# ylsung/vl-merging

Hardware: AMD Instinct MI355X
Metric: VL samples/sec (fwd+bwd) base_vl 384^2 at 1/2/4/8 GPUs; merge GB/s vs HBM peak (higher is better)
Workload: dtype bf16

## Files before the change

### include/vlm_hip.h

```cpp
#ifndef VLM_HIP_H
#define VLM_HIP_H
#include <stddef.h>
#include <stdint.h>

#ifdef __cplusplus
extern "C" {
#endif

#define VLM_OK 0
#define VLM_ERR_ARG (-1)
#define VLM_ERR_LAUNCH (-2)
#define VLM_ERR_WORKSPACE (-3)
#define VLM_ERR_UNSUPPORTED (-4)

#define VLM_ABI_VERSION 11
int vlm_abi_version(void);
int vlm_device_cus(void);
int vlm_set_cu_budget(int cus);
int vlm_debug_occupy(int workgroups, int threads, int lds_bytes, int microseconds, void* stream);

#define VLM_MERGE_LERP 0
#define VLM_MERGE_TASKVEC 1
#define VLM_MERGE_MEAN 2
#define VLM_MERGE_MAX_SRC 4
// ... 197 lines not shown
  uint64_t chunks_off;
  uint64_t first_off;
  uint64_t records_off;
  uint64_t results_off;
} vlm_stock_header_t;
#define VLM_STOCK_SUMS (VLM_MERGE_MAX_SRC + VLM_PAIRSTATS_PAIRS)

typedef struct {
  double sq[VLM_MERGE_MAX_SRC];
  double dot[6];
  double cos_pair[6];
  double cos;
  double t;
  float scale;
  uint32_t reserved;
} vlm_stock_result_t;

size_t vlm_stock_plan_bytes(int n_jobs, uint64_t total_elems);
int vlm_stock_plan_upload(const vlm_stock_job_t* jobs_host, int n_jobs, void* workspace, size_t workspace_bytes, void* stream);
int vlm_stock_run(void* workspace, void* stream);

typedef struct {
  void* dst;
  const void* base;
  const void* src[VLM_MERGE_MAX_SRC];
  uint64_t k;
  uint64_t n_elem;
  int32_t n_src;
  float lam;
} vlm_sce_job_t;

typedef struct {
  uint64_t n_jobs, n_units, n_chunks;
  uint64_t jobs_off;
  uint64_t chunks_off;
  uint64_t unit0_off;
  uint64_t units_off;
  uint64_t state_off;
  uint64_t counters_off;
  uint64_t hist_off;
  uint64_t first_off;
  uint64_t records_off;
} vlm_sce_header_t;
typedef struct {
  uint32_t key;
  uint32_t reserved;
  uint64_t rank;
  double sq[VLM_MERGE_MAX_SRC];
  double tot;
  float w[VLM_MERGE_MAX_SRC];
} vlm_sce_result_t;
#define VLM_SCE_COUNTERS 3

size_t vlm_sce_plan_bytes(int n_jobs, uint64_t total_elems);
int vlm_sce_plan_upload(const vlm_sce_job_t* jobs_host, int n_jobs, void* workspace, size_t workspace_bytes, void* stream);
int vlm_sce_run(void* workspace, void* stream);

#define VLM_ACT_NONE 0
#define VLM_ACT_GELU 1
#define VLM_ACT_GELU_BWD 2
#define VLM_ACT_GELU_DERIV 3
#define VLM_ACT_MUL_AUX 4

typedef struct {
  const float* bias;
  const float* col_scale;
  const float* row_scale;
  const float* residual;
  int64_t ld_res;
  void* aux;
  int64_t ld_aux;
  int32_t act;
  float alpha;
  int32_t accumulate;
  int32_t reserved;
  float* col_sum;
  float* col_sum_ws;
  float* splitk_ws;
  uint64_t splitk_ws_bytes;
} vlm_epilogue_t;

int vlm_gemm_bf16(int ta, int tb, int M, int N, int K, const void* A, int lda, const void* B, int ldb, void* C,
                  int ldc, int c_is_f32, const vlm_epilogue_t* epi, void* stream);
#define VLM_GEMM_MAX_GROUPS 4
typedef struct {
  int32_t row0, rows;
  const void* B;
  int32_t ldb;
  int32_t reserved;
  const float* bias;
  float* col_sum;
  float* col_sum_ws;
} vlm_gemm_group_t;
int vlm_gemm_bf16_grouped(int n_groups, const vlm_gemm_group_t* groups, int N, int K, const void* A, int lda, void* C,
                          int ldc, int c_is_f32, const vlm_epilogue_t* epi, void* stream);
typedef struct {
  int32_t row0, rows;
  float* C;
  int32_t accumulate;
  int32_t reserved;
} vlm_wgrad_group_t;
int vlm_gemm_wgrad_grouped(int n_groups, const vlm_wgrad_group_t* groups, int M, int N, const void* A, int lda,
                           const void* B, int ldb, int ldc, float* splitk_ws, uint64_t splitk_ws_bytes, void* stream);
typedef struct {
  const void* dy;
  int32_t ld_dy, M;
  const void* x;
  int32_t ld_x, N;
  float* dW;
  int32_t ldc, accumulate;
} vlm_wgrad_problem_t;
int vlm_gemm_wgrad_batch(int n, const vlm_wgrad_problem_t* problems, int T, float* splitk_ws, uint64_t splitk_ws_bytes,
                         void* stream);
int vlm_gemm_set_big_tile_mode(int mode);

int vlm_layernorm_fwd(const float* x, int ldx, int M, int D, const float* gamma, const float* beta, float eps,
                      void* y, int ldy, int y_is_f32, float* stats, void* stream);
#define VLM_ROW_WS_BYTES(D) ((size_t)1536 * 2 * (size_t)(D) * sizeof(float))
int vlm_layernorm_bwd(const void* dy, int lddy, int dy_is_f32, const float* x, int ldx, const float* stats,
                      const float* gamma, int M, int D, const float* dres, int lddres, float* dx, int lddx,
                      float* dgamma, float* dbeta, float* workspace, size_t workspace_bytes, int* deferred_blocks,
                      void* stream);
typedef struct {
  const void* y;
  int32_t ldy;
  const float* gamma;
  const float* row_scale;
  void* dy;
  int32_t lddy;
  float* dgamma;
  float* dbias;
  float* workspace;
  size_t workspace_bytes;
} vlm_layerscale_t;
int vlm_layernorm_bwd_scale(const void* dy, int lddy, int dy_is_f32, const float* x, int ldx, const float* stats,
                            const float* gamma, int M, int D, const float* dres, int lddres, float* dx, int lddx,
                            float* dgamma, float* dbeta, float* workspace, size_t workspace_bytes,
                            const vlm_layerscale_t* scale, int* deferred_blocks, void* stream);
#define VLM_MAX_FOLD_JOBS 16
typedef struct {
  const float* partials;
  int32_t nblocks;
  int32_t D;
  float* out0;
  float* out1;
} vlm_fold_job_t;
int vlm_colreduce_batch(const vlm_fold_job_t* jobs_host, int n_jobs, void* stream);
int vlm_layerscale_bwd(const float* dx, int lddx, const void* y_bf16, int ldy, const float* gamma,
                       const float* row_scale, int M, int D, void* dy_bf16, int lddy, float* dgamma, float* dbias,
                       float* workspace, size_t workspace_bytes, int* deferred_blocks, void* stream);
#define VLM_MAX_LAYERSCALE_JOBS 32
typedef struct {
  const float* weight;
  const float* gamma;
  const float* bias;
  void* shadow;
  float* bias_out;
  float* raw_w;
  float* raw_b;
  float* dweight;
  float* dbias;
  float* dgamma;
  int32_t N, K;
} vlm_layerscale_job_t;
int vlm_layerscale_fold(const vlm_layerscale_job_t* jobs_host, int n_jobs, void* stream);
int vlm_layerscale_finish(const vlm_layerscale_job_t* jobs_host, int n_jobs, void* stream);
// ... 35 lines not shown
int vlm_weighted_sum(const float* const* terms, const float* weights, int count, float* out, void* stream);

typedef struct {
  const void* g;
  int g_is_f32;
  int ld;
  int first_row, row_step, count;
} vlm_scatter_src_t;
int vlm_scatter_rows(void* dx, int dx_is_f32, int ld_dx, int R, int D, const vlm_scatter_src_t* src, int n_src, void* stream);

int vlm_adamw_step(float* p, float* g, float* m, float* v, void* p_bf16, uint64_t n, float lr, float beta1,
                   float beta2, float eps, float weight_decay, float step_size, float grad_scale, int zero_grad,
                   void* stream);
int vlm_cast_f32_bf16(const float* src, void* dst_bf16, uint64_t n, void* stream);
int vlm_embedding_bwd(const float* gy, int ld, const int64_t* ids, int64_t n, int D, int64_t padding_idx, float* dW, int ld_w,
                      int64_t vocab, void* stream);
typedef struct {
  uint64_t src;
  uint64_t dst;
  int32_t rows, cols;
  int32_t tile_row, tile_col;
} vlm_transpose_tile_t;
int vlm_transpose_bf16_tiles(const vlm_transpose_tile_t* tiles_dev, int n_tiles, void* stream);

int vlm_droppath_rows(const float* u, float keep, int B, int n0, int n1, int base0, int base1, float* out, void* stream);
int vlm_droppath_sites(const float* u0, const float* u1, const float* keep, int n_sites, int B, int n0, int n1, int base0,
                       int base1, int rows, float* out, void* stream);
int vlm_patch_im2col(const float* image, void* patches_bf16, int B, int H, int W, int P, int lead_rows, void* stream);
int vlm_accumulate_f32_f64(const float* src, double* dst_f64, uint64_t n, void* stream);
int vlm_gram_f64(const void* x, int ldx, int M, int D, int x_is_f32, double* gram, void* stream);
int vlm_gemm_f64(int ta, int tb, int M, int N, int K, double alpha, const void* A, int lda, int a_is_f32, const double* B,
                 int ldb, double beta, double* C, int ldc, void* stream);
int vlm_scale_gram_f64(const double* src, double* dst, int n, double alpha, int accumulate, void* stream);
int vlm_cholesky_f64(double* A, int n, int* status, void* stream);
int vlm_solve_spd_right_f64(const double* chol, int n, double* rhs, int ld, int rows, void* stream);
int vlm_gemm_f64_batched(int ta, int tb, int M, int N, int K, double alpha, const void* const* A_list, int lda, int a_is_f32,
                         const double* const* B_list, int ldb, double beta, double* const* C_list, int ldc, int count, void* stream);
int vlm_cholesky_f64_batched(double* const* A_list, int count, int n, int* status, void* stream);
int vlm_solve_spd_right_f64_batched(double* const* chol_list, int n, double* const* rhs_list, int ld, int rows, int count, void* stream);

#define VLM_ATTN_JOINT 0
#define VLM_ATTN_SEPARATE 1

typedef struct {
  const void* qkv;
  int32_t ld_qkv;
  int32_t H;
  int32_t total_rows;
  int32_t R;
  const float* bias_t;
  const int16_t* rel_index;
  const int16_t* rel_index_t;
  int32_t ld_index;
  int32_t index_rows;
  int32_t ld_index_t;
  int32_t index_t_rows;
  int32_t head_row0;
  int32_t mode;
  const uint8_t* keep0;
  const uint8_t* keep1;
  int32_t B, n0, n1, base0, base1, pos1;
  float scale;
  int32_t reserved;
  const void* bias_dense;
  const void* bias_dense_t;
  int32_t dense_tiles;
  int32_t reserved2;
} vlm_attn_desc_t;

size_t vlm_bias_dense_bytes(int n0, int n1, int pos1, int mode);
int vlm_bias_dense(const float* bias_t, int n_cols, int R, const int16_t* index, int ld_index, int n0, int n1, int pos1,
                   int mode, int k_major, void* out_f16, void* stream);

int vlm_attention_fwd(const vlm_attn_desc_t* d, void* out_bf16, int ld_out, float* lse, void* stream);
typedef struct {
  float* dq[2];
  float* dv[2];
} vlm_attn_colsum_t;

size_t vlm_attention_bwd_ws_floats(const vlm_attn_desc_t* d, int with_dbias);
int vlm_attention_bwd(const vlm_attn_desc_t* d, const void* out_bf16, int ld_out, const void* dout_bf16, int ld_dout,
                      const float* lse, float* delta_ws, size_t ws_floats, void* dqkv_bf16, int ld_dqkv, float* dbias_t,
                      const vlm_attn_colsum_t* colsum, void* stream);

#ifdef __cplusplus
}
#endif
#endif
```

### vl-merging_amd/_lib.py

```python
import ctypes
import os

_HERE = os.path.dirname(os.path.abspath(__file__))
LIB_PATH = os.environ.get("VLM_LIB_PATH") or os.path.join(_HERE, "lib", "libvlm_hip.so")
_lib = None

c_void_p = ctypes.c_void_p
c_int = ctypes.c_int
c_float = ctypes.c_float
c_size_t = ctypes.c_size_t
c_u64 = ctypes.c_uint64

MERGE_LERP, MERGE_TASKVEC, MERGE_MEAN = 0, 1, 2
MERGE_MAX_SRC = 4


class MergeJob(ctypes.Structure):
    _fields_ = [
        ("dst", c_void_p),
        ("base", c_void_p),
        ("src", c_void_p * MERGE_MAX_SRC),
        ("ratio", c_float * MERGE_MAX_SRC),
        ("n_src", ctypes.c_int32),
        ("mode", ctypes.c_int32),
# ... 215 lines not shown
                ("N", ctypes.c_int32), ("dW", c_void_p), ("ldc", ctypes.c_int32), ("accumulate", ctypes.c_int32)]


class FoldJob(ctypes.Structure):
    _fields_ = [("partials", c_void_p), ("nblocks", ctypes.c_int32), ("D", ctypes.c_int32), ("out0", c_void_p),
                ("out1", c_void_p)]


class LayerScale(ctypes.Structure):
    _fields_ = [("y", c_void_p), ("ldy", ctypes.c_int32), ("gamma", c_void_p), ("row_scale", c_void_p), ("dy", c_void_p),
                ("lddy", ctypes.c_int32), ("dgamma", c_void_p), ("dbias", c_void_p), ("workspace", c_void_p),
                ("workspace_bytes", c_size_t)]


class AttnColsum(ctypes.Structure):
    _fields_ = [("dq", c_void_p * 2), ("dv", c_void_p * 2)]


ACT_NONE, ACT_GELU, ACT_GELU_BWD, ACT_GELU_DERIV, ACT_MUL_AUX = 0, 1, 2, 3, 4
ATTN_JOINT, ATTN_SEPARATE = 0, 1


class AttnDesc(ctypes.Structure):
    _fields_ = [
        ("qkv", c_void_p), ("ld_qkv", ctypes.c_int32), ("H", ctypes.c_int32), ("total_rows", ctypes.c_int32),
        ("R", ctypes.c_int32), ("bias_t", c_void_p), ("rel_index", c_void_p), ("rel_index_t", c_void_p),
        ("ld_index", ctypes.c_int32), ("index_rows", ctypes.c_int32), ("ld_index_t", ctypes.c_int32),
        ("index_t_rows", ctypes.c_int32), ("head_row0", ctypes.c_int32), ("mode", ctypes.c_int32),
        ("keep0", c_void_p), ("keep1", c_void_p),
        ("B", ctypes.c_int32), ("n0", ctypes.c_int32), ("n1", ctypes.c_int32), ("base0", ctypes.c_int32),
        ("base1", ctypes.c_int32), ("pos1", ctypes.c_int32), ("scale", c_float), ("reserved", ctypes.c_int32),
        ("bias_dense", c_void_p), ("bias_dense_t", c_void_p), ("dense_tiles", ctypes.c_int32), ("reserved2", ctypes.c_int32),
    ]


class LayerScaleJob(ctypes.Structure):
    _fields_ = [("weight", c_void_p), ("gamma", c_void_p), ("bias", c_void_p), ("shadow", c_void_p), ("bias_out", c_void_p),
                ("raw_w", c_void_p), ("raw_b", c_void_p), ("dweight", c_void_p), ("dbias", c_void_p), ("dgamma", c_void_p),
                ("N", ctypes.c_int32), ("K", ctypes.c_int32)]


MAX_LAYERSCALE_JOBS = 32


class VlmError(RuntimeError):
    pass


_ERR = {-1: "VLM_ERR_ARG", -2: "VLM_ERR_LAUNCH", -3: "VLM_ERR_WORKSPACE", -4: "VLM_ERR_UNSUPPORTED"}

SIGNATURES = {
    "vlm_abi_version": (c_int, []),
    "vlm_device_cus": (c_int, []),
    "vlm_set_cu_budget": (c_int, [c_int]),
    "vlm_debug_occupy": (c_int, [c_int, c_int, c_int, c_int, c_void_p]),
    "vlm_layerscale_fold": (c_int, [ctypes.POINTER(LayerScaleJob), c_int, c_void_p]),
    "vlm_layerscale_finish": (c_int, [ctypes.POINTER(LayerScaleJob), c_int, c_void_p]),
    "vlm_merge_plan_bytes": (c_size_t, [c_int, c_u64]),
    "vlm_merge_plan_upload": (c_int, [ctypes.POINTER(MergeJob), c_int, c_void_p, c_size_t, c_void_p]),
    "vlm_merge_run": (c_int, [c_void_p, c_void_p]),
    "vlm_ties_plan_bytes": (c_size_t, [c_int, c_u64]),
    "vlm_ties_plan_upload": (c_int, [ctypes.POINTER(TiesJob), c_int, c_void_p, c_size_t, c_void_p]),
    "vlm_ties_run": (c_int, [c_void_p, c_void_p]),
    "vlm_dare_plan_bytes": (c_size_t, [c_int, c_u64]),
    "vlm_dare_plan_upload": (c_int, [ctypes.POINTER(DareJob), c_int, c_void_p, c_size_t, c_void_p]),
    "vlm_dare_run": (c_int, [c_void_p, c_void_p]),
    "vlm_band_plan_bytes": (c_size_t, [c_int, c_u64]),
    "vlm_band_plan_upload": (c_int, [ctypes.POINTER(BandJob), c_int, c_void_p, c_size_t, c_void_p]),
    "vlm_band_run": (c_int, [c_void_p, c_void_p]),
    "vlm_della_plan_bytes": (c_size_t, [c_int, c_u64]),
    "vlm_della_plan_upload": (c_int, [ctypes.POINTER(DellaJob), c_int, c_void_p, c_size_t, c_void_p]),
    "vlm_della_run": (c_int, [c_void_p, c_void_p]),
    "vlm_pairstats_plan_bytes": (c_size_t, [c_int, c_u64]),
    "vlm_pairstats_plan_upload": (c_int, [ctypes.POINTER(PairStatsJob), c_int, c_void_p, c_size_t, c_void_p]),
    "vlm_pairstats_run": (c_int, [c_void_p, c_void_p]),
    "vlm_stock_plan_bytes": (c_size_t, [c_int, c_u64]),
    "vlm_stock_plan_upload": (c_int, [ctypes.POINTER(StockJob), c_int, c_void_p, c_size_t, c_void_p]),
    "vlm_stock_run": (c_int, [c_void_p, c_void_p]),
    "vlm_sce_plan_bytes": (c_size_t, [c_int, c_u64]),
    "vlm_sce_plan_upload": (c_int, [ctypes.POINTER(SceJob), c_int, c_void_p, c_size_t, c_void_p]),
    "vlm_sce_run": (c_int, [c_void_p, c_void_p]),
    "vlm_gemm_bf16": (c_int, [c_int, c_int, c_int, c_int, c_int, c_void_p, c_int, c_void_p, c_int, c_void_p, c_int,
                              c_int, ctypes.POINTER(Epilogue), c_void_p]),
    "vlm_gemm_bf16_grouped": (c_int, [c_int, ctypes.POINTER(GemmGroup), c_int, c_int, c_void_p, c_int, c_void_p, c_int, c_int,
                                      ctypes.POINTER(Epilogue), c_void_p]),
    "vlm_gemm_wgrad_grouped": (c_int, [c_int, ctypes.POINTER(WgradGroup), c_int, c_int, c_void_p, c_int, c_void_p, c_int, c_int,
                                       c_void_p, c_u64, c_void_p]),
    "vlm_gemm_wgrad_batch": (c_int, [c_int, ctypes.POINTER(WgradProblem), c_int, c_void_p, c_u64, c_void_p]),
    "vlm_attention_fwd": (c_int, [ctypes.POINTER(AttnDesc), c_void_p, c_int, c_void_p, c_void_p]),
    "vlm_attention_bwd_ws_floats": (c_size_t, [ctypes.POINTER(AttnDesc), c_int]),
    "vlm_attention_bwd": (c_int, [ctypes.POINTER(AttnDesc), c_void_p, c_int, c_void_p, c_int, c_void_p, c_void_p, c_size_t,
                                  c_void_p, c_int, c_void_p, c_void_p, c_void_p]),
    "vlm_layernorm_fwd": (c_int, [c_void_p, c_int, c_int, c_int, c_void_p, c_void_p, c_float, c_void_p, c_int, c_int,
                                  c_void_p, c_void_p]),
    "vlm_layernorm_bwd": (c_int, [c_void_p, c_int, c_int, c_void_p, c_int, c_void_p, c_void_p, c_int, c_int, c_void_p,
                                  c_int, c_void_p, c_int, c_void_p, c_void_p, c_void_p, c_size_t,
                                  ctypes.POINTER(c_int), c_void_p]),
    "vlm_layernorm_bwd_scale": (c_int, [c_void_p, c_int, c_int, c_void_p, c_int, c_void_p, c_void_p, c_int, c_int, c_void_p,
                                        c_int, c_void_p, c_int, c_void_p, c_void_p, c_void_p, c_size_t,
                                        ctypes.POINTER(LayerScale), ctypes.POINTER(c_int), c_void_p]),
    "vlm_layerscale_bwd": (c_int, [c_void_p, c_int, c_void_p, c_int, c_void_p, c_void_p, c_int, c_int, c_void_p, c_int,
                                   c_void_p, c_void_p, c_void_p, c_size_t, ctypes.POINTER(c_int), c_void_p]),
    "vlm_colreduce_batch": (c_int, [ctypes.POINTER(FoldJob), c_int, c_void_p]),
    "vlm_gemm_set_big_tile_mode": (c_int, [c_int]),
    "vlm_colsum_bf16": (c_int, [c_void_p, c_int, c_int, c_int, c_void_p, c_void_p]),
    "vlm_adamw_step": (c_int, [c_void_p, c_void_p, c_void_p, c_void_p, c_void_p, c_u64, c_float, c_float, c_float,
                               c_float, c_float, c_float, c_float, c_int, c_void_p]),
    "vlm_accumulate_f32_f64": (c_int, [c_void_p, c_void_p, c_u64, c_void_p]),
    "vlm_gram_f64": (c_int, [c_void_p, c_int, c_int, c_int, c_int, c_void_p, c_void_p]),
    "vlm_gemm_f64": (c_int, [c_int, c_int, c_int, c_int, c_int, ctypes.c_double, c_void_p, c_int, c_int, c_void_p, c_int,
                             ctypes.c_double, c_void_p, c_int, c_void_p]),
    "vlm_scale_gram_f64": (c_int, [c_void_p, c_void_p, c_int, ctypes.c_double, c_int, c_void_p]),
    "vlm_cholesky_f64": (c_int, [c_void_p, c_int, c_void_p, c_void_p]),
    "vlm_solve_spd_right_f64": (c_int, [c_void_p, c_int, c_void_p, c_int, c_int, c_void_p]),
    "vlm_gemm_f64_batched": (c_int, [c_int, c_int, c_int, c_int, c_int, ctypes.c_double, ctypes.POINTER(c_void_p), c_int, c_int,
                                     ctypes.POINTER(c_void_p), c_int, ctypes.c_double, ctypes.POINTER(c_void_p), c_int, c_int, c_void_p]),
    "vlm_cholesky_f64_batched": (c_int, [ctypes.POINTER(c_void_p), c_int, c_int, c_void_p, c_void_p]),
    "vlm_solve_spd_right_f64_batched": (c_int, [ctypes.POINTER(c_void_p), c_int, ctypes.POINTER(c_void_p), c_int, c_int, c_int, c_void_p]),
    "vlm_cross_entropy_fwd": (c_int, [c_void_p, c_int, c_int, c_int, c_void_p, ctypes.c_int64, c_void_p, c_void_p, c_void_p]),
    "vlm_cross_entropy_bwd": (c_int, [c_void_p, c_int, c_int, c_int, c_void_p, ctypes.c_int64, c_void_p, c_void_p, c_void_p, c_int,
                                      c_void_p]),
    "vlm_l2norm_fwd": (c_int, [c_void_p, c_int, c_int, c_int, c_int, c_void_p, c_void_p, c_void_p]),
    "vlm_l2norm_bwd": (c_int, [c_void_p, c_void_p, c_void_p, c_int, c_int, c_void_p, c_int, c_int, c_void_p]),
    "vlm_contrastive_ws_floats": (c_size_t, [c_int]),
    "vlm_contrastive": (c_int, [c_void_p, c_void_p, c_int, c_int, c_int, c_void_p, c_void_p, c_void_p, c_void_p, c_void_p, c_void_p,
                                c_void_p]),
    "vlm_small_cross_entropy": (c_int, [c_void_p, c_int, c_int, c_int, c_int, c_void_p, c_void_p, c_void_p, c_void_p]),
    "vlm_cross_entropy_reduce": (c_int, [c_void_p, c_void_p, c_int, c_int, ctypes.c_int64, c_void_p, c_void_p]),
    "vlm_scale_by_scalar": (c_int, [ctypes.POINTER(c_void_p), ctypes.POINTER(c_void_p), ctypes.POINTER(c_int), c_int, c_void_p, c_void_p]),
    "vlm_text_rows_fwd": (c_int, [c_void_p, c_int, c_void_p, c_int, c_void_p, c_void_p, c_void_p, c_float, c_void_p, c_float, c_float,
                                  c_void_p, c_void_p, c_int, c_void_p, c_int, c_void_p]),
    "vlm_text_rows_bwd_ws_floats": (c_size_t, [c_int]),
    "vlm_text_rows_bwd": (c_int, [c_void_p, c_int, c_void_p, c_int, c_void_p, c_int, c_void_p, c_void_p, c_void_p, c_void_p, c_float, c_float,
                                  c_int, c_void_p, ctypes.c_int64, c_void_p, c_void_p, c_void_p, c_void_p, c_void_p, c_void_p]),
    "vlm_image_rows_prep": (c_int, [c_void_p, c_void_p, c_void_p, c_int, c_void_p, c_void_p]),
    "vlm_image_lead_rows": (c_int, [c_void_p, c_int, c_int, c_int, c_int, c_void_p, c_void_p]),
    "vlm_image_rows_bwd_ws_floats": (c_size_t, [c_int]),
    "vlm_image_rows_bwd": (c_int, [c_void_p, c_int, c_int, c_int, c_int, c_void_p, c_void_p, c_void_p, c_void_p, c_void_p, c_void_p]),
    "vlm_tanh_fwd": (c_int, [c_void_p, c_int, c_int, c_int, c_void_p, c_void_p]),
    "vlm_act_bwd": (c_int, [c_void_p, c_int, c_int, c_void_p, c_int, c_int, c_int, c_int, c_int, c_void_p, c_void_p]),
    "vlm_colsum_small": (c_int, [c_void_p, c_int, c_int, c_int, c_void_p, c_void_p]),
    "vlm_sample_negatives": (c_int, [c_void_p, c_int, c_int, c_void_p, c_int, c_int, c_int, c_int, c_void_p, c_void_p, c_void_p]),
    "vlm_weighted_sum": (c_int, [ctypes.POINTER(c_void_p), ctypes.POINTER(c_float), c_int, c_void_p, c_void_p]),
    "vlm_scatter_rows": (c_int, [c_void_p, c_int, c_int, c_int, c_int, c_void_p, c_int, c_void_p]),
    "vlm_cast_f32_bf16": (c_int, [c_void_p, c_void_p, c_u64, c_void_p]),
    "vlm_embedding_bwd": (c_int, [c_void_p, c_int, c_void_p, ctypes.c_int64, c_int, ctypes.c_int64, c_void_p, c_int,
                                  ctypes.c_int64, c_void_p]),
    "vlm_bias_dense_bytes": (c_size_t, [c_int, c_int, c_int, c_int]),
    "vlm_bias_dense": (c_int, [c_void_p, c_int, c_int, c_void_p, c_int, c_int, c_int, c_int, c_int, c_int, c_void_p,
                               c_void_p]),
    "vlm_transpose_bf16_tiles": (c_int, [c_void_p, c_int, c_void_p]),
    "vlm_droppath_sites": (c_int, [c_void_p, c_void_p, c_void_p, c_int, c_int, c_int, c_int, c_int, c_int, c_int, c_void_p,
                                   c_void_p]),
    "vlm_droppath_rows": (c_int, [c_void_p, c_float, c_int, c_int, c_int, c_int, c_int, c_void_p, c_void_p]),
    "vlm_patch_im2col": (c_int, [c_void_p, c_void_p, c_int, c_int, c_int, c_int, c_int, c_void_p]),
}


def get_lib():
    global _lib
    if _lib is None:
        if not os.path.exists(LIB_PATH):
            raise VlmError(
                f"{LIB_PATH} is missing: build it with `python -c 'import __graft_entry__ as g; g.build()'` "
                "(hipcc --offload-arch=gfx950).  There is no CPU fallback for the hot path.")
        import torch
        lib = ctypes.CDLL(LIB_PATH)
        for name, (res, args) in SIGNATURES.items():
            fn = getattr(lib, name)
            fn.restype = res
            fn.argtypes = args
        _lib = lib
    return _lib


# ... 19 lines not shown
```

### vl-merging_amd/csrc/attention_bwd.hip

```cpp
#include "vlm_common.h"
#include "attention_common.h"
#include "vlm_diag.h"

struct attn_bwd_params_t {
  attn_params_t f;
  const bf16_t* d_o;
  int ld_do;
  const float* lse;
  const bf16_t* o;
  int ld_o;
  float* delta;
  float inv_c1;
  bf16_t* dqkv;
  int ld_dqkv;
  float* dbias_t;
  float* nstat;
  float* dq_colsum[2];
  float* dv_colsum[2];
};

#include "attention_bwd_dkvb.h"
#include "attention_bwd_dq2.h"

template <bool HAS_BIAS>
__global__ __launch_bounds__(ATT_THREADS, 2) void attn_bwd_dq_kernel(const attn_bwd_params_t bp) {
  const attn_params_t& p = bp.f;
  __shared__ __attribute__((aligned(16))) unsigned char smem[6 * ATT_TILE_BYTES + 512];
  unsigned char* ldsK = smem;
  unsigned char* ldsKt = smem + 2 * ATT_TILE_BYTES;
  unsigned char* ldsV = smem + 4 * ATT_TILE_BYTES;
  float* kmask = reinterpret_cast<float*>(smem + 6 * ATT_TILE_BYTES);

  const int tid = threadIdx.x, lane = tid & 63;
  const int wave = __builtin_amdgcn_readfirstlane(tid >> 6);
  const int r = lane & 31, hh = lane >> 5;
  const att_pos_t ps = att_pos(p.seq);
  int wtile, b, h;
  if (!att_work_item(att_num_tiles(ps.n0, ps.n1, ps.pos1, p.mode), ps.B, p.H, wtile, b, h)) return;
  const att_span_t sp = att_span(ps, p.mode, wtile);
  const int D = p.H * 64;
  const int qp = sp.p0 + wave * 32 + r;
  const int qrow_raw = qp < sp.s_hi ? att_row_of(ps, b, qp) : -1;
  const bool qvalid = qrow_raw >= 0;
  const size_t qrow = qvalid ? (size_t)qrow_raw : (size_t)att_row_of(ps, b, sp.s_lo);
  const int ntiles = (sp.s_hi - sp.s_lo + ATT_BK - 1) / ATT_BK;
  const float c1 = p.scale * ATT_LOG2E;

  bf16x8 qf[4], dof[4];
  {
    const bf16_t* qptr = p.qkv + qrow * p.ld_qkv + h * 64 + 8 * hh;
    const bf16_t* dptr = bp.d_o + qrow * bp.ld_do + h * 64 + 8 * hh;
#pragma unroll
    for (int s = 0; s < 4; ++s) {
      const bf16x8 raw = *reinterpret_cast<const bf16x8*>(qptr + 16 * s);
#pragma unroll
      for (int j = 0; j < 8; ++j) qf[s][j] = (bf16_t)((float)raw[j] * c1);
      dof[s] = *reinterpret_cast<const bf16x8*>(dptr + 16 * s);
    }
  }
  f32x16 neglse, negdel;
  {
    const bf16_t* optr = bp.o + qrow * bp.ld_o + h * 64 + 8 * hh;
    float part = 0.f;
#pragma unroll
    for (int s = 0; s < 4; ++s) {
      const bf16x8 raw = *reinterpret_cast<const bf16x8*>(optr + 16 * s);
#pragma unroll
      for (int j = 0; j < 8; ++j) part += (float)raw[j] * (float)dof[s][j];
    }
    part += att_other_half(part);
    const size_t at = (size_t)h * p.total_rows + qrow;
    const float lse2 = qvalid ? bp.lse[at] : INFINITY;
    if (qvalid && hh == 0) {
      bp.delta[at] = part;
      if (bp.nstat) {
        bp.nstat[at] = -lse2 * bp.inv_c1;
        bp.nstat[(size_t)p.H * p.total_rows + at] = -part;
      }
    }
    const float l2 = -lse2;
    const float dl = qvalid ? -part : 0.f;
#pragma unroll
    for (int i = 0; i < 16; ++i) { neglse[i] = l2; negdel[i] = dl; }
  }
  f16x8 sel0, sel1;
  att_select_frags(lane, sel0, sel1);
  const __amdgpu_buffer_rsrc_t rkv = __builtin_amdgcn_make_buffer_rsrc(
      const_cast<bf16_t*>(p.qkv), 0, (uint32_t)((size_t)p.total_rows * p.ld_qkv * 2), 0x00020000);
  const att_dense_layout_t dl = att_dense_layout(ps.n0, ps.n1, ps.pos1, p.mode);
  const __amdgpu_buffer_rsrc_t rbias = __builtin_amdgcn_make_buffer_rsrc(
      const_cast<_Float16*>(HAS_BIAS ? p.dense + (size_t)(p.head_row0 + h) * p.dense_tiles * 2048 : nullptr), 0,
      HAS_BIAS ? (uint32_t)p.dense_tiles * 4096u : 0, 0x00020000);
  const uint32_t bvoff = att_bias_voff(dl, sp.part, sp.tile_in_part * 4 + wave, lane);

  f32x16 o[2];
#pragma unroll
  for (int i = 0; i < 16; ++i) o[0][i] = o[1][i] = 0.f;

  auto tile_masked = [&](int kp0) {
    return (p.keep0 != nullptr && kp0 < ps.n0) || (p.keep1 != nullptr && kp0 + ATT_BK > ps.pos1) ||
           (!HAS_BIAS && (kp0 < ps.pos1 || kp0 + ATT_BK > sp.s_hi));
  };
// ... 559 lines not shown
#pragma unroll
      for (int j = 0; j < 16; ++j)
        atomicAdd(reinterpret_cast<unsigned long long*>(smem + 2 * ids[j]), (unsigned long long)(long long)(acc[j] * FIX));
    }
  }
  __syncthreads();
  float* g = bp.dbias_t + (size_t)(p.head_row0 + h) * p.R;
  for (int i = tid; i < p.R; i += ATT_DB16_THREADS) {
    const long long v = (long long)hist64[i];
    if (v != 0) atomicAdd(g + i, (float)v * UNFIX);
  }
}

static int att_dbias_pairs(const attn_params_t& p) {
  if (p.mode == VLM_ATTN_SEPARATE) {
    const int a = (p.seq.n0 + ATT_BQ - 1) / ATT_BQ, c = (p.seq.n1 + ATT_BQ - 1) / ATT_BQ;
    return a * a + c * c;
  }
  const int a = (p.seq.pos1 + p.seq.n1 + ATT_BQ - 1) / ATT_BQ;
  return a * a;
}
static int att_dbias_groups(const attn_params_t& p, int pairs, int cus) {
  int groups = 1;
  float best = 1e30f;
  for (int g = 1; g <= 8 && g <= p.seq.B && pairs > 0; ++g) {
    const float item = 2.2f * (float)p.seq.B / (float)g + 10.0f;
    const float t = ((float)pairs * p.H * g / (float)cus + 0.5f) * item;
    if (t < best) { best = t; groups = g; }
  }
  return groups;
}

struct att_bwd_plan_t {
  bool dq2;
  int W;
  int panel_blocks;
  size_t lds;
  int groups, items;
  size_t nstat_off;
  size_t ws_floats;
};
static att_bwd_plan_t att_bwd_plan(const attn_params_t& p, bool want_dbias) {
  const size_t hr = (size_t)p.H * p.total_rows;
  att_bwd_plan_t pl = {p.bias_t && att_handplaced_covers(p), 0, 0, 0, 1, 0, 0, hr};
  if (!want_dbias) return pl;
  int cus = vlm_device_cus();
  if (cus <= 0) cus = 256;
  for (int W = 8; W >= 4 && !pl.W && p.dense_t && p.idx; W -= 4) {
    pl.lds = dkvb_lds_bytes(p, W, pl.panel_blocks);
    if (pl.lds) pl.W = W;
  }
  if (pl.W) {
    const dkvb_geom_t gm = dkvb_geom(p.seq.n0, p.seq.n1, p.seq.pos1, p.mode);
    const int nkb = gm.nkb[0] + gm.nkb[1];
    const int rounds = (p.seq.B + pl.W - 1) / pl.W;
    int g = cus / (nkb * p.H > 0 ? nkb * p.H : 1);
    if (g > rounds) g = rounds;
    pl.groups = g < 1 ? 1 : g;
    pl.items = nkb * p.H * pl.groups;
    return pl;
  }
  const int pairs = att_dbias_pairs(p);
  pl.groups = att_dbias_groups(p, pairs, cus);
  pl.items = pairs * p.H * pl.groups;
  pl.nstat_off = hr;
  pl.ws_floats = 3 * hr;
  return pl;
}

extern "C" size_t vlm_attention_bwd_ws_floats(const vlm_attn_desc_t* d, int with_dbias) {
  (void)with_dbias;
  attn_params_t p;
  if (att_fill_params(d, p) != VLM_OK) return 0;
  return att_bwd_plan(p, p.bias_t != nullptr).ws_floats;
}

template <int W>
static void dkvb_launch(const attn_bwd_params_t& bp, const att_bwd_plan_t& pl, hipStream_t s) {
  static const hipError_t asked = hipFuncSetAttribute((const void*)attn_bwd_dkvb_kernel<W>, hipFuncAttributeMaxDynamicSharedMemorySize, 160 * 1024);
  (void)asked;
  hipLaunchKernelGGL((attn_bwd_dkvb_kernel<W>), dim3((unsigned)((pl.items + 7) / 8 * 8)), dim3(W * 64), pl.lds, s, bp, pl.groups, pl.panel_blocks);
}

extern "C" int vlm_attention_bwd(const vlm_attn_desc_t* d, const void* out, int ld_out, const void* d_out,
                                 int ld_dout, const float* lse, float* delta_ws, size_t ws_floats, void* dqkv, int ld_dqkv,
                                 float* dbias_t, const vlm_attn_colsum_t* colsum, void* stream) {
  attn_bwd_params_t bp;
  int rc = att_fill_params(d, bp.f);
  if (rc != VLM_OK) return rc;
  if (!out || !d_out || !lse || !delta_ws || !dqkv) return VLM_ERR_ARG;
  if ((ld_out & 7) || (ld_dout & 7) || (ld_dqkv & 3) || ((uintptr_t)out & 15) || ((uintptr_t)d_out & 15))
    return VLM_ERR_ARG;
  if (bp.f.bias_t && (!bp.f.idx || (bp.f.ld_idx & 3))) return VLM_ERR_ARG;
  attn_params_t& p = bp.f;
  const int nt0 = (p.seq.n0 + ATT_BQ - 1) / ATT_BQ, nt1 = (p.seq.n1 + ATT_BQ - 1) / ATT_BQ;
  if (nt0 + nt1 == 0 || p.seq.B == 0) return VLM_OK;
  hipStream_t s = (hipStream_t)stream;
  bp.d_o = reinterpret_cast<const bf16_t*>(d_out);
  bp.ld_do = ld_dout;
  bp.lse = lse;
  bp.delta = delta_ws;
  bp.dqkv = reinterpret_cast<bf16_t*>(dqkv);
  bp.ld_dqkv = ld_dqkv;
  bp.dbias_t = dbias_t;
  for (int sgm = 0; sgm < 2; ++sgm) {
    bp.dq_colsum[sgm] = colsum ? colsum->dq[sgm] : nullptr;
    bp.dv_colsum[sgm] = colsum ? colsum->dv[sgm] : nullptr;
  }

  if ((size_t)p.total_rows * p.ld_qkv * 2 >= (1ull << 32) || (size_t)p.total_rows * ld_dout * 2 >= (1ull << 32)) return VLM_ERR_UNSUPPORTED;
  if (p.bias_t && (!p.dense || !p.dense_t)) return VLM_ERR_ARG;
  if (p.dense && p.dense_tiles != att_dense_layout(p.seq.n0, p.seq.n1, p.seq.pos1, p.mode).tiles) return VLM_ERR_ARG;
  if (p.bias_t && dbias_t && ((size_t)p.R * 8 + 8 > 2 * (size_t)(8 * ATT_TILE_BYTES + 1024) || !p.idx_t)) return VLM_ERR_UNSUPPORTED;
  const att_bwd_plan_t pl = att_bwd_plan(p, p.bias_t && dbias_t);
  if (ws_floats < pl.ws_floats) return VLM_ERR_WORKSPACE;
  bp.nstat = pl.nstat_off ? delta_ws + pl.nstat_off : nullptr;
  bp.o = reinterpret_cast<const bf16_t*>(out);
  bp.ld_o = ld_out;
  bp.inv_c1 = 1.0f / (p.scale * ATT_LOG2E);

  const int nt = att_num_tiles(p.seq.n0, p.seq.n1, p.seq.pos1, p.mode);
  dim3 grid(att_grid_size(nt, p.seq.B, p.H)), block(ATT_THREADS);
  if (p.bias_t) {
    if (pl.dq2) hipLaunchKernelGGL(attn_bwd_dq2_kernel, grid, block, 0, s, bp);
    else hipLaunchKernelGGL((attn_bwd_dq_kernel<true>), grid, block, 0, s, bp);
    VLM_CHECK_LAUNCH();
    if (pl.W == 8) dkvb_launch<8>(bp, pl, s);
    else if (pl.W == 4) dkvb_launch<4>(bp, pl, s);
    else hipLaunchKernelGGL((attn_bwd_dkv_kernel<true>), grid, block, 0, s, bp);
    if (!pl.W && dbias_t) {
      VLM_CHECK_LAUNCH();
      hipLaunchKernelGGL(attn_bwd_dbias16_kernel, dim3((unsigned)((pl.items + 7) / 8 * 8)), dim3(ATT_DB16_THREADS), 0, s, bp, pl.groups);
    }
  } else {
    hipLaunchKernelGGL((attn_bwd_dq_kernel<false>), grid, block, 0, s, bp);
    VLM_CHECK_LAUNCH();
    hipLaunchKernelGGL((attn_bwd_dkv_kernel<false>), grid, block, 0, s, bp);
  }
  VLM_CHECK_LAUNCH();
  return VLM_OK;
}
```

### vl-merging_amd/csrc/attention_bwd_dkvb.h

```cpp
#pragma once

#define ATT_KB 32

__device__ __forceinline__ uint32_t dkvb_off(uint32_t row, uint32_t ch) {
  const uint32_t f = ((row >> 2) & 3u) | (((row >> 1) & 1u) << 2);
  return row * 128u + ((ch ^ f) << 4);
}

struct dkvb_geom_t {
  int nkb[2];
};
static inline __host__ __device__ dkvb_geom_t dkvb_geom(int n0, int n1, int pos1, int mode) {
  dkvb_geom_t g;
  if (mode == VLM_ATTN_SEPARATE) { g.nkb[0] = (n0 + ATT_KB - 1) / ATT_KB; g.nkb[1] = (n1 + ATT_KB - 1) / ATT_KB; }
  else { g.nkb[0] = (pos1 + n1 + ATT_KB - 1) / ATT_KB; g.nkb[1] = 0; }
  return g;
}
static inline __host__ __device__ int dkvb_nblk(int n0, int n1, int pos1, int mode, int part) {
  if (mode == VLM_ATTN_SEPARATE) return ((part ? n1 : n0) + ATT_KB - 1) / ATT_KB;
  return (pos1 + n1 + ATT_KB - 1) / ATT_KB;
}

typedef __attribute__((address_space(3))) s16x4 dkvb_lds_s16x4;

// ... 1 lines not shown
__device__ __forceinline__ bf16x8 dkvb_pack8(const f32x16& v, int first) {
  dkvb_f32x8 t;
#pragma unroll
  for (int i = 0; i < 8; ++i) t[i] = v[first + i];
  return __builtin_convertvector(t, bf16x8);
}

template <int W>
__global__ __launch_bounds__(W * 64, 1) void attn_bwd_dkvb_kernel(const attn_bwd_params_t bp, int n_groups, int panel_blocks) {
  const attn_params_t& p = bp.f;
  extern __shared__ __attribute__((aligned(1024))) unsigned char dkvb_smem[];
  float* panel = reinterpret_cast<float*>(dkvb_smem);
  unsigned char* slots = dkvb_smem + (size_t)panel_blocks * 4096;

  const int tid = threadIdx.x, lane = tid & 63;
  const int wave = __builtin_amdgcn_readfirstlane(tid >> 6);
  const int r = lane & 31, hh = lane >> 5;
  const att_pos_t ps = att_pos(p.seq);
  const int D = p.H * 64;
  const dkvb_geom_t gm = dkvb_geom(ps.n0, ps.n1, ps.pos1, p.mode);
  const int NKB = gm.nkb[0] + gm.nkb[1];
  const int total = NKB * p.H * n_groups, per = (total + 7) >> 3;
  const int logical = (blockIdx.x & 7) * per + (blockIdx.x >> 3);
  if ((int)(blockIdx.x >> 3) >= per || logical >= total) return;
  const int kbi = logical % NKB;
  const int grp = (logical / NKB) % n_groups;
  const int h = logical / (NKB * n_groups);
  const int part = kbi >= gm.nkb[0] ? 1 : 0;
  const int sb = part ? kbi - gm.nkb[0] : kbi;
  int s_lo, s_hi;
  if (p.mode == VLM_ATTN_SEPARATE) { s_lo = part ? ps.pos1 : 0; s_hi = part ? ps.NP : ps.n0; }
  else { s_lo = 0; s_hi = ps.NP; }
  const int kp0 = s_lo + sb * ATT_KB;
  const int nblk = (s_hi - s_lo + ATT_KB - 1) / ATT_KB;
  const int b_lo = (int)((long)ps.B * grp / n_groups), b_hi = (int)((long)ps.B * (grp + 1) / n_groups);
  const int wact = nblk < W ? nblk : W;
  const int S = nblk / wact;
  const float c1 = p.scale * ATT_LOG2E;

  const int kp = kp0 + r;
  const bool kvalid = kp < s_hi && (kp < ps.n0 || kp >= ps.pos1);
  const bool ktext = kp < ps.n0;
  const uint8_t* keepk = ktext ? p.keep0 : p.keep1;
  const int keep_at = ktext ? kp : kp - ps.pos1, keep_n = ktext ? ps.n0 : ps.n1;
  const int krow0 = ktext ? ps.base0 + kp : ps.base1 + (kp - ps.pos1), kstr = ktext ? ps.n0 : ps.n1;
  f16x8 sel0, sel1;
  att_select_frags(lane, sel0, sel1);
  const att_dense_layout_t dl = att_dense_layout(ps.n0, ps.n1, ps.pos1, p.mode);
  const __amdgpu_buffer_rsrc_t rbias = __builtin_amdgcn_make_buffer_rsrc(
      const_cast<_Float16*>(p.dense_t + (size_t)(p.head_row0 + h) * p.dense_tiles * 2048), 0, (uint32_t)p.dense_tiles * 4096u, 0x00020000);
  const uint32_t bvoff = att_bias_voff(dl, part, sb, lane);
  const __amdgpu_buffer_rsrc_t rq = __builtin_amdgcn_make_buffer_rsrc(
      const_cast<bf16_t*>(p.qkv), 0, (uint32_t)((size_t)p.total_rows * p.ld_qkv * 2), 0x00020000);
  const __amdgpu_buffer_rsrc_t rdo = __builtin_amdgcn_make_buffer_rsrc(
      const_cast<bf16_t*>(bp.d_o), 0, (uint32_t)((size_t)p.total_rows * bp.ld_do * 2), 0x00020000);
  const __amdgpu_buffer_rsrc_t rlse = __builtin_amdgcn_make_buffer_rsrc(
      const_cast<float*>(bp.lse + (size_t)h * p.total_rows), 0, (uint32_t)p.total_rows * 4u, 0x00020000);
  const __amdgpu_buffer_rsrc_t rdel = __builtin_amdgcn_make_buffer_rsrc(
      const_cast<float*>(bp.delta + (size_t)h * p.total_rows), 0, (uint32_t)p.total_rows * 4u, 0x00020000);

  const uint32_t c16 = (uint32_t)(lane & 7) * 16u + (uint32_t)h * 128u;
  const uint32_t voff_q = (uint32_t)(lane >> 3) * (uint32_t)(p.ld_qkv * 2) + c16, voff_o = (uint32_t)(lane >> 3) * (uint32_t)(bp.ld_do * 2) + c16;
  unsigned char* slot = slots + wave * 8192;
  const uint32_t wr_off0 = dkvb_off(lane >> 3, lane & 7), wr_off1 = dkvb_off(8 + (lane >> 3), lane & 7);
  const uint32_t row_off0 = dkvb_off(r, hh);
  uint32_t tr_off[2][2];
  {
    const int g16 = (lane >> 4) & 1, qq = (lane & 15) >> 2, pp = lane & 3;
#pragma unroll
    for (int db = 0; db < 2; ++db)
#pragma unroll
      for (int hi = 0; hi < 2; ++hi)
        tr_off[db][hi] = dkvb_off(8 * hi + 4 * hh + qq, 2 * (db * 2 + g16) + (pp >> 1)) + 8 * (pp & 1);
  }

  for (int i = tid; i < nblk * 256; i += W * 64) reinterpret_cast<f32x4*>(panel)[i] = (f32x4){0.f, 0.f, 0.f, 0.f};
  __syncthreads();

  float cs_t[2] = {0.f, 0.f}, cs_i[2] = {0.f, 0.f};

  const int rounds = (b_hi - b_lo + wact - 1) / wact;
  for (int rd = 0; rd < rounds; ++rd) {
    const int b = b_lo + rd * wact + wave;
    const bool active = wave < wact && b < b_hi;

    bf16x8 kf[4], vf[4], bstat;
    f32x16 dk[2], dv[2];
#pragma unroll
    for (int i = 0; i < 16; ++i) dk[0][i] = dk[1][i] = dv[0][i] = dv[1][i] = 0.f;
#pragma unroll
    for (int j = 0; j < 8; ++j) bstat[j] = (bf16_t)0.f;
    u32x4 nq[4], no_[4], nbw[2];
    float nlse = 0.f, ndel = 0.f;
    const uint32_t row_txt = (uint32_t)(ps.base0 + b * ps.n0), row_img = (uint32_t)(ps.base1 + b * ps.n1 - ps.pos1);
    auto row_of = [&](int qp) -> uint32_t {
      qp = qp < s_hi - 1 ? qp : s_hi - 1;
      return (uint32_t)qp + (qp < ps.n0 ? row_txt : row_img);
    };
    auto request = [&](int j) {
      const int q0 = s_lo + j * ATT_KB;
      if (q0 >= ps.pos1 && q0 + ATT_KB <= s_hi) {
        const uint32_t row0 = row_img + (uint32_t)q0;
#pragma unroll
        for (int u = 0; u < 4; ++u) {
          nq[u] = __builtin_bit_cast(u32x4, __builtin_amdgcn_raw_buffer_load_b128(rq, voff_q, (row0 + 8u * u) * (uint32_t)(p.ld_qkv * 2), 0));
          no_[u] = __builtin_bit_cast(u32x4, __builtin_amdgcn_raw_buffer_load_b128(rdo, voff_o, (row0 + 8u * u) * (uint32_t)(bp.ld_do * 2), 0));
        }
        nlse = __builtin_bit_cast(float, __builtin_amdgcn_raw_buffer_load_b32(rlse, (uint32_t)r * 4u, row0 * 4u, 0));
        ndel = __builtin_bit_cast(float, __builtin_amdgcn_raw_buffer_load_b32(rdel, (uint32_t)r * 4u, row0 * 4u, 0));
      } else {
#pragma unroll
        for (int u = 0; u < 4; ++u) {
          const uint32_t row = row_of(q0 + 8 * u + (lane >> 3));
          nq[u] = __builtin_bit_cast(u32x4, __builtin_amdgcn_raw_buffer_load_b128(rq, row * (uint32_t)(p.ld_qkv * 2) + c16, 0, 0));
          no_[u] = __builtin_bit_cast(u32x4, __builtin_amdgcn_raw_buffer_load_b128(rdo, row * (uint32_t)(bp.ld_do * 2) + c16, 0, 0));
        }
        const uint32_t row = row_of(q0 + r);
        nlse = __builtin_bit_cast(float, __builtin_amdgcn_raw_buffer_load_b32(rlse, row * 4u, 0, 0));
        ndel = __builtin_bit_cast(float, __builtin_amdgcn_raw_buffer_load_b32(rdel, row * 4u, 0, 0));
      }
      {
        const uint32_t soff = (uint32_t)(j >> 1) * 4096u + (uint32_t)(j & 1) * 2048u;
        nbw[0] = __builtin_bit_cast(u32x4, __builtin_amdgcn_raw_buffer_load_b128(rbias, bvoff, soff, 0));
        nbw[1] = __builtin_bit_cast(u32x4, __builtin_amdgcn_raw_buffer_load_b128(rbias, bvoff + 1024, soff, 0));
      }
    };
    if (active) {
      const size_t krow = (size_t)(krow0 + b * kstr);
      const bf16_t* kptr = p.qkv + (kvalid ? krow : (size_t)0) * p.ld_qkv + D + h * 64 + 8 * hh;
#pragma unroll
      for (int s = 0; s < 4; ++s) {
        const bf16x8 raw = *reinterpret_cast<const bf16x8*>(kptr + 16 * s);
#pragma unroll
        for (int j = 0; j < 8; ++j) kf[s][j] = (bf16_t)(kvalid ? (float)raw[j] * c1 : 0.f);
        vf[s] = *reinterpret_cast<const bf16x8*>(kptr + D + 16 * s);
      }
      const bool kept = kvalid && (!keepk || keepk[(size_t)b * keep_n + keep_at] != 0);
      if (hh == 0) {
        bstat[0] = bstat[1] = bstat[2] = (bf16_t)1.0f;
        bstat[3] = (bf16_t)(kept ? 0.f : ATT_NEG_BIG);
      }
      request(wave * S);
    }

    if (!active) {
      for (int t = 0, ph = 0; t < nblk; ++t) {
        if (++ph == S || t + 1 == nblk) { ph = 0; __syncthreads(); }
      }
      continue;
    }
    for (int t = 0, ph = 0, j = wave * S; t < nblk; ++t) {
#pragma unroll
      for (int u = 0; u < 4; ++u) {
        const uint32_t wo = (u & 1 ? wr_off1 : wr_off0) + (u >> 1) * 2048u;
        *reinterpret_cast<u32x4*>(slot + wo) = nq[u];
        *reinterpret_cast<u32x4*>(slot + 4096 + wo) = no_[u];
      }
      bf16x8 astat_e, astat_d;
      {
        const int qp = s_lo + j * ATT_KB + r;
        const bool qok = qp < s_hi && (qp < ps.n0 || qp >= ps.pos1);
        const float ve = qok ? -nlse : ATT_NEG_BIG, vd = qok ? -ndel : 0.f;
        const bf16_t e0 = (bf16_t)ve, d0 = (bf16_t)vd;
        const bf16_t e1 = (bf16_t)(ve - (float)e0), d1 = (bf16_t)(vd - (float)d0);
        const bf16_t z = (bf16_t)0.f;
        const bool lo = hh == 0;
        astat_e = (bf16x8){lo ? e0 : z, lo ? e1 : z, z, lo ? (bf16_t)1.0f : z, z, z, z, z};
// ... 147 lines not shown
```

### vl-merging_amd/csrc/attention_bwd_dq2.h

```cpp
#pragma once

#define DQ2_STAGE 8192
#define DQ2_KM (4 * DQ2_STAGE)
#define DQ2_LDS (DQ2_KM + 1024)

typedef __attribute__((ext_vector_type(16))) unsigned dq2_u32x16;
typedef __attribute__((ext_vector_type(8))) unsigned dq2_u32x8;

#define DQ2_CLOBBER_V \
  "v88", "v89", "v90", "v91", "v92", "v93", "v94", "v95", "v96", "v97", "v98", "v99", "v100", "v101", "v102", "v103", "v104", \
  "v105", "v106", "v107", "v108", "v109", "v110", "v111", "v112", "v113", "v114", "v115", "v116", "v117", "v118", "v119",       \
  "v120", "v121", "v122", "v123", "v124", "v125", "v126", "v127", "v128", "v129", "v130", "v131", "v132", "v133", "v134",       \
  "v135", "v136", "v137", "v138", "v139", "v140", "v141", "v142", "v143", "v144", "v145", "v146", "v147", "v148", "v149",       \
  "v150", "v151", "v152", "v153", "v154", "v155", "v156", "v157", "v158", "v159", "v168", "v169", "v170", "v171", "v172", "v173", "v174", "v175", "v184", "v185", "v186", "v187",       \
  "v196", "v197", "v198", "v199", "v200", "v201"

__device__ __forceinline__ void dq2_split3(float x, uint32_t& hi, uint32_t& mid, uint32_t& lo) {
  const bf16_t h = (bf16_t)x;
  const float r1 = x - (float)h;
  const bf16_t m = (bf16_t)r1;
  const bf16_t l = (bf16_t)(r1 - (float)m);
  hi = (uint32_t)__builtin_bit_cast(unsigned short, h);
  mid = (uint32_t)__builtin_bit_cast(unsigned short, m);
  lo = (uint32_t)__builtin_bit_cast(unsigned short, l);
}

__global__ __launch_bounds__(ATT_THREADS, 2) void attn_bwd_dq2_kernel(const attn_bwd_params_t bp) {
  const attn_params_t& p = bp.f;
  __shared__ __attribute__((aligned(16))) unsigned char lds[DQ2_LDS > 128 * 68 * 4 ? DQ2_LDS : 128 * 68 * 4];

  const int tid = threadIdx.x, lane = tid & 63;
  const int wave = __builtin_amdgcn_readfirstlane(tid >> 6);
  const int r = lane & 31, hh = lane >> 5;
  const att_pos_t ps = att_pos(p.seq);
  int wtile, b, h;
  if (!att_work_item(att_num_tiles(ps.n0, ps.n1, ps.pos1, p.mode), ps.B, p.H, wtile, b, h)) return;
  const att_span_t sp = att_span(ps, p.mode, wtile);
  ATT_STAMP(0);
  const int D = p.H * 64;
  const int ntiles = (sp.s_hi - sp.s_lo + ATT_BK - 1) / ATT_BK;
  const uint32_t lds0 = (uint32_t)(uintptr_t)(att_lds_void*)lds;
  const __amdgpu_buffer_rsrc_t rkv = __builtin_amdgcn_make_buffer_rsrc(
      const_cast<bf16_t*>(p.qkv), 0, (uint32_t)((size_t)p.total_rows * p.ld_qkv * 2), 0x00020000);
  const att_dense_layout_t dl = att_dense_layout(ps.n0, ps.n1, ps.pos1, p.mode);
  const uint32_t bvoff = att_bias_voff(dl, sp.part, sp.tile_in_part * 4 + wave, lane);
  const uint32_t rb_bytes = (uint32_t)p.dense_tiles * 4096u;
  const _Float16* bias_col = p.dense + (size_t)(p.head_row0 + h) * p.dense_tiles * 2048;
  const __amdgpu_buffer_rsrc_t rbias = __builtin_amdgcn_make_buffer_rsrc(const_cast<_Float16*>(bias_col), 0, rb_bytes, 0x00020000);

  u32x4 b0w[2], b1w[2];
  b0w[0] = __builtin_bit_cast(u32x4, __builtin_amdgcn_raw_buffer_load_b128(rbias, bvoff, 0, 0));
  b0w[1] = __builtin_bit_cast(u32x4, __builtin_amdgcn_raw_buffer_load_b128(rbias, bvoff + 1024, 0, 0));
  b1w[0] = __builtin_bit_cast(u32x4, __builtin_amdgcn_raw_buffer_load_b128(rbias, bvoff + 2048, 0, 0));
  b1w[1] = __builtin_bit_cast(u32x4, __builtin_amdgcn_raw_buffer_load_b128(rbias, bvoff + 3072, 0, 0));
  const int qp = sp.p0 + wave * 32 + r;
  const int qrow_raw = qp < sp.s_hi ? att_row_of(ps, b, qp) : -1;
  const bool qvalid = qrow_raw >= 0;
  const size_t qrow = qvalid ? (size_t)qrow_raw : (size_t)att_row_of(ps, b, sp.s_lo);
  bf16x8 rawq[4], dof[4], rawo[4];
  {
    const bf16_t* qptr = p.qkv + qrow * p.ld_qkv + h * 64 + 8 * hh;
    const bf16_t* dptr = bp.d_o + qrow * bp.ld_do + h * 64 + 8 * hh;
    const bf16_t* optr = bp.o + qrow * bp.ld_o + h * 64 + 8 * hh;
#pragma unroll
    for (int ss = 0; ss < 4; ++ss) {
      rawq[ss] = *reinterpret_cast<const bf16x8*>(qptr + 16 * ss);
      dof[ss] = *reinterpret_cast<const bf16x8*>(dptr + 16 * ss);
      rawo[ss] = *reinterpret_cast<const bf16x8*>(optr + 16 * ss);
    }
  }
  const size_t stat_at = (size_t)h * p.total_rows + qrow;
  const float lse_raw = bp.lse[stat_at];
  const int mpos = sp.s_lo + (tid >> 6) * ATT_BK + (tid & 63);
  const bool mtxt = mpos < ps.n0, mimg = mpos >= ps.pos1 && mpos < ps.NP;
  const bool mok = tid < 128 && (mtxt || mimg) && mpos < sp.s_hi;
  const __amdgpu_buffer_rsrc_t rkeep0 = __builtin_amdgcn_make_buffer_rsrc(
      const_cast<uint8_t*>(p.keep0 ? p.keep0 : reinterpret_cast<const uint8_t*>(p.qkv)), 0, p.keep0 ? (uint32_t)(ps.B * ps.n0) : 0u, 0x00020000);
  const uint32_t keep_raw = (uint32_t)(uint8_t)__builtin_amdgcn_raw_buffer_load_b8(rkeep0, (mok && mtxt) ? (uint32_t)(b * ps.n0 + mpos) : 0xFFFFFFF0u, 0, 0);

  const uint32_t drow = (uint32_t)wave * 8u + (uint32_t)(lane >> 3), c16 = lane & 7;
  const uint32_t fsw = ((drow >> 2) & 3u) | (((drow >> 1) & 1u) << 2);
  const uint32_t voff = (drow * p.ld_qkv + ((c16 ^ fsw) << 3)) * 2u;
  auto stage_block = [&](int blk) {
    const int kp0 = sp.s_lo + blk * 32, pq = kp0 + (int)drow;
    const bool txt = pq < ps.n0, img = pq >= ps.pos1 && pq < ps.NP;
    const bool ok = (txt || img) && pq < sp.s_hi;
    const int first = txt ? ps.base0 + b * ps.n0 + kp0 : ps.base1 + b * ps.n1 + (kp0 - ps.pos1);
    const uint32_t rowoff = (uint32_t)first * (uint32_t)p.ld_qkv * 2u;
    const uint32_t kcol = (uint32_t)(D + h * 64) * 2u, vcol = (uint32_t)(2 * D + h * 64) * 2u;
    unsigned char* dst = lds + (blk & 3) * DQ2_STAGE + wave * 1024;
    __builtin_amdgcn_raw_ptr_buffer_load_lds(rkv, (att_lds_void*)dst, 16, ok ? rowoff + kcol + voff : 0xFFFFFFF0u, 0, 0, 0);
    __builtin_amdgcn_raw_ptr_buffer_load_lds(rkv, (att_lds_void*)(dst + 4096), 16, ok ? rowoff + vcol + voff : 0xFFFFFFF0u, 0, 0, 0);
  };
  stage_block(0);
  stage_block(1);
  stage_block(2);

  {
    uint32_t w = 0u;
    if (tid < 128) w = ((mok && !(mtxt && p.keep0 && keep_raw == 0)) ? 0u : 0xC6EAu) | 0x3F800000u;
    else if (tid < 192) w = 0x3F800000u;
    *reinterpret_cast<uint32_t*>(lds + DQ2_KM + tid * 4) = w;
  }
  const float c1 = p.scale * ATT_LOG2E;
  dq2_u32x16 qv, dov;
#pragma unroll
  for (int ss = 0; ss < 4; ++ss) {
    bf16x8 sc;
#pragma unroll
    for (int j = 0; j < 8; ++j) sc[j] = (bf16_t)((float)rawq[ss][j] * c1);
    const u32x4 wq = __builtin_bit_cast(u32x4, sc), wd = __builtin_bit_cast(u32x4, dof[ss]);
#pragma unroll
    for (int e = 0; e < 4; ++e) { qv[4 * ss + e] = wq[e]; dov[4 * ss + e] = wd[e]; }
  }
  dq2_u32x8 stats;
  {
    float part = 0.f;
#pragma unroll
    for (int ss = 0; ss < 4; ++ss)
#pragma unroll
      for (int j = 0; j < 8; ++j) part += (float)rawo[ss][j] * (float)dof[ss][j];
// ... 131 lines not shown
```

### vl-merging_amd/csrc/gemm.hip

```cpp
#include "vlm_common.h"
#include "vlm_diag.h"
#include "wgrad_plan.h"
#include <atomic>

#define GEMM_BM 128
#define GEMM_BN 128
#define GEMM_BK 64
#define GEMM_THREADS 256
#define GEMM_TILE_BYTES (GEMM_BM * GEMM_BK * 2)

typedef __attribute__((address_space(3))) s16x4 lds_s16x4;

__device__ __forceinline__ float gelu_cdf(float x, float& ez2) {
  const float t = __builtin_amdgcn_rcpf(fmaf(0.3275911f * 0.70710678118654752440f, fabsf(x), 1.0f));
  ez2 = __builtin_amdgcn_exp2f((x * x) * (-0.5f * 1.4426950408889634f));
  float poly = fmaf(t, 0.5f * 1.061405429f, 0.5f * -1.453152027f);
  poly = fmaf(t, poly, 0.5f * 1.421413741f);
  poly = fmaf(t, poly, 0.5f * -0.284496736f);
  poly = fmaf(t, poly, 0.5f * 0.254829592f);
  const float e = fmaf(-(poly * t), ez2, 0.5f);
  return 0.5f + copysignf(e, x);
}
__device__ __forceinline__ float gelu_erf(float x) {
  float ez2;
// ... 31 lines not shown
    r[u] = __builtin_amdgcn_raw_buffer_load_b128(rsrc, off, 0, 0);
  }
}

template <bool KSTRIDED>
__device__ __forceinline__ void stage_store(const u32x4 (&r)[4], unsigned char* lds, int tid) {
#pragma unroll
  for (int u = 0; u < 4; ++u) {
    const uint32_t p = tid + 256 * u;
    uint32_t byte;
    if (!KSTRIDED) {
      const uint32_t row = p >> 3, chunk = p & 7;
      byte = row * 128 + ((chunk ^ (row & 7)) << 4);
    } else {
      const uint32_t krow = p >> 4, c16 = p & 15;
      const uint32_t c32 = (c16 >> 1) ^ (krow & 3) ^ (((krow >> 3) & 1) << 2);
      byte = krow * 256 + c32 * 32 + (c16 & 1) * 16;
    }
    *reinterpret_cast<u32x4*>(lds + byte) = r[u];
  }
}

typedef __attribute__((address_space(3))) void lds_void;
__device__ __forceinline__ void stage_dma(__amdgpu_buffer_rsrc_t rsrc, unsigned char* tile, uint32_t row0, uint32_t k0,
                                          uint32_t ld, int wave, int lane) {
#pragma unroll
  for (int u = 0; u < 4; ++u) {
    const int j = wave + 4 * u;
    const uint32_t row = j * 8 + (lane >> 3), chunk = (lane & 7) ^ (row & 7);
    const uint32_t off = ((row0 + row) * ld + k0 + chunk * 8) * 2;
    __builtin_amdgcn_raw_ptr_buffer_load_lds(rsrc, (lds_void*)(tile + j * 1024), 16, off, 0, 0, 0);
  }
}

template <bool KSTRIDED>
__device__ __forceinline__ bf16x8 frag_load(const unsigned char* lds, int xblk , int ksub,
                                            int lane) {
  if (!KSTRIDED) {
    const uint32_t row = xblk * 16 + (lane & 15);
    const uint32_t chunk = ksub * 4 + (lane >> 4);
    const uint32_t byte = row * 128 + ((chunk ^ (row & 7)) << 4);
    return *reinterpret_cast<const bf16x8*>(lds + byte);
  } else {
    const uint32_t g = lane >> 4, q = (lane & 15) >> 2, p = lane & 3;
    const uint32_t row = ksub * 32 + 8 * g + q;
    const uint32_t c32 = ((uint32_t)xblk ^ q ^ ((g & 1) << 2));
    const uint32_t byte = row * 256 + c32 * 32 + 8 * p;
    s16x4 lo = __builtin_amdgcn_ds_read_tr16_b64_v4i16((lds_s16x4*)(lds + byte));
    s16x4 hi = __builtin_amdgcn_ds_read_tr16_b64_v4i16((lds_s16x4*)(lds + byte + 4 * 256));
    s16x8 v = {lo[0], lo[1], lo[2], lo[3], hi[0], hi[1], hi[2], hi[3]};
    return __builtin_bit_cast(bf16x8, v);
  }
}

struct gemm_group_t {
  const void* B;
  const float* bias;
  float* col_sum;
  float* col_sum_ws;
  int ldb, row0, row_end, tile0;
};

struct gemmT_group_t {
  const void* A;
  const void* B;
  int lda, ldb, M, N, tiles_n, ntile;
  int row0, row_end, item0, kps;
  uint32_t ws_base;
};

struct gemm_params_t {
  const void* A;
  const void* B;
  void* C;
  int M, N, K;
  int lda, ldb, ldc;
  vlm_epilogue_t epi;
  int tiles_m, tiles_n;
  int group_m;
  int splits, ksteps_per_split;
  int n_groups;
  gemm_group_t grp[VLM_GEMM_MAX_GROUPS];
  gemmT_group_t grpT[VLM_GEMM_MAX_GROUPS];
  VLM_DIAG_GEMM_FIELD
};

__device__ __forceinline__ void lane16_swap(float& x, float& y) {
  asm volatile("s_nop 1\n\tv_permlane16_swap_b32 %0, %1" : "+v"(x), "+v"(y));
}

template <bool OUT_F32, bool LEAN = false>
__device__ __forceinline__ int gemm_epilogue(const gemm_params_t& p, const f32x4 (&acc)[4][4], int mw0, int nw0, int lane,
                                             float* red = nullptr, int red_off = 0) {
  const vlm_epilogue_t& e = p.epi;
  const bool vec_ok = ((p.ldc & 3) == 0) && (!e.aux || (e.ld_aux & 3) == 0) && (!e.residual || (e.ld_res & 3) == 0);
  const bool vec8_ok = vec_ok && (OUT_F32 || (p.ldc & 7) == 0) && (!e.aux || ((e.ld_aux & 7) == 0 && ((uintptr_t)e.aux & 15) == 0)) &&
                       (!e.residual || ((uintptr_t)e.residual & 15) == 0) && (!e.bias || ((uintptr_t)e.bias & 15) == 0) &&
                       (!e.col_scale || ((uintptr_t)e.col_scale & 15) == 0);
  if (vec8_ok && mw0 + 64 <= p.M && nw0 + 64 <= p.N) {
    const bool has_res = e.residual != nullptr, bwd = e.act == VLM_ACT_GELU_BWD || e.act == VLM_ACT_MUL_AUX, accum = OUT_F32 && e.accumulate;
    const int g = lane >> 4;
    const int nl = nw0 + (g & 1) * 16 + (g >> 1) * 8;
    float bia[2][8], gam[2][8], csum[2][8];
#pragma unroll
    for (int jp = 0; jp < 2; ++jp)
#pragma unroll
      for (int r = 0; r < 8; ++r) csum[jp][r] = 0.f;
#define EPI_LOAD_COL_VECTORS()                                                                                          \
  _Pragma("unroll") for (int jp = 0; jp < 2; ++jp) _Pragma("unroll") for (int q = 0; q < 2; ++q) {                    \
    const f32x4 b4 = e.bias ? *reinterpret_cast<const f32x4*>(e.bias + nl + jp * 32 + q * 4) : (f32x4){0.f, 0.f, 0.f, 0.f}; \
    const f32x4 g4 =                                                                                                    \
        e.col_scale ? *reinterpret_cast<const f32x4*>(e.col_scale + nl + jp * 32 + q * 4) : (f32x4){1.f, 1.f, 1.f, 1.f}; \
    _Pragma("unroll") for (int r = 0; r < 4; ++r) {                                                                     \
      bia[jp][q * 4 + r] = b4[r];                                                                                       \
      gam[jp][q * 4 + r] = g4[r];                                                                                       \
    }                                                                                                                   \
  }
    if (!LEAN) { EPI_LOAD_COL_VECTORS() }
#pragma unroll
    for (int hf = 0; hf < 4; ++hf) {
      f32x4 rsd[1][2][2], old[1][2][2];
      bf16x8 hx[1][2];
      float rs[1];
      if (LEAN) { EPI_LOAD_COL_VECTORS() }
#pragma unroll
      for (int ii = 0; ii < 1; ++ii) {
        const size_t m = mw0 + (hf + ii) * 16 + (lane & 15);
        rs[ii] = e.row_scale ? e.row_scale[m] : 1.0f;
#pragma unroll
        for (int jp = 0; jp < 2; ++jp) {
          const int n = nl + jp * 32;
          if (has_res) {
            rsd[ii][jp][0] = *reinterpret_cast<const f32x4*>(e.residual + m * e.ld_res + n);
            rsd[ii][jp][1] = *reinterpret_cast<const f32x4*>(e.residual + m * e.ld_res + n + 4);
          }
          if (bwd) hx[ii][jp] = *reinterpret_cast<const bf16x8*>(reinterpret_cast<const bf16_t*>(e.aux) + m * e.ld_aux + n);
          if (accum) {
            old[ii][jp][0] = *reinterpret_cast<const f32x4*>(reinterpret_cast<const float*>(p.C) + m * p.ldc + n);
            old[ii][jp][1] = *reinterpret_cast<const f32x4*>(reinterpret_cast<const float*>(p.C) + m * p.ldc + n + 4);
          }
        }
      }
#pragma unroll
      for (int ii = 0; ii < 1; ++ii) {
        const size_t m = mw0 + (hf + ii) * 16 + (lane & 15);
#pragma unroll
        for (int jp = 0; jp < 2; ++jp) {
          const int n = nl + jp * 32;
          float v[8];
#pragma unroll
          for (int r = 0; r < 4; ++r) {
            float x = acc[hf + ii][2 * jp][r] * e.alpha, y = acc[hf + ii][2 * jp + 1][r] * e.alpha;
            lane16_swap(x, y);
            v[r] = x;
            v[4 + r] = y;
          }
#pragma unroll
          for (int r = 0; r < 8; ++r) v[r] += bia[jp][r];
          if (bwd) {
#pragma unroll
            for (int r = 0; r < 8; ++r) v[r] *= act_bwd_factor(e.act, (float)hx[ii][jp][r]);
          } else if (e.act == VLM_ACT_GELU_DERIV) {
            bf16x8 h;
#pragma unroll
            for (int r = 0; r < 8; ++r) {
              float dg;
// ... 489 lines not shown
#pragma unroll
        for (int r = 0; r < 8; ++r) atomicAdd(e.col_sum + n + r, csum[r]);
      }
    }
  }
};

#define EPIL_DUMP_ROW(A0, A1, II, OFF)                                                           \
  _Pragma("unroll") for (int j = 0; j < 4; ++j) {                                                \
    *reinterpret_cast<f32x4*>(wr + (OFF) + 64 * j) = A0[II][j];                                  \
    *reinterpret_cast<f32x4*>(wr + (OFF) + 64 * (4 + j)) = A1[II][j];                            \
  }
#define BIG_EPILOGUE_LOOP_DEEP(AHEAD)                                                                             \
  unsigned char* wr = wl + (lane & 15) * EPIL_PITCH + (lane >> 4) * 16;                                            \
  epil_in_t in8[8];                                                                                                \
  _Pragma("unroll") for (int b8 = 0; b8 < (AHEAD); ++b8) ep.load_inputs(in8[b8], b8);                              \
  _Pragma("unroll") for (int q = 0; q < 4; ++q) {                                                                  \
    switch (q) {                                                                                                   \
      case 0: EPIL_DUMP_ROW(acc00, acc01, 0, 0) EPIL_DUMP_ROW(acc00, acc01, 1, 16 * EPIL_PITCH) break;             \
      case 1: EPIL_DUMP_ROW(acc00, acc01, 2, 0) EPIL_DUMP_ROW(acc00, acc01, 3, 16 * EPIL_PITCH) break;             \
      case 2: EPIL_DUMP_ROW(acc10, acc11, 0, 0) EPIL_DUMP_ROW(acc10, acc11, 1, 16 * EPIL_PITCH) break;             \
      default: EPIL_DUMP_ROW(acc10, acc11, 2, 0) EPIL_DUMP_ROW(acc10, acc11, 3, 16 * EPIL_PITCH) break;            \
    }                                                                                                              \
    ep.process(in8[2 * q], 2 * q, 0);                                                                              \
    if (2 * q + (AHEAD) < 8) ep.load_inputs(in8[2 * q + (AHEAD)], 2 * q + (AHEAD));                                \
    ep.process(in8[2 * q + 1], 2 * q + 1, 16 * EPIL_PITCH);                                                        \
    if (2 * q + 1 + (AHEAD) < 8) ep.load_inputs(in8[2 * q + 1 + (AHEAD)], 2 * q + 1 + (AHEAD));                    \
  }
#define BIG_EPILOGUE_LOOP()                                                                                       \
  unsigned char* wr = wl + (lane & 15) * EPIL_PITCH + (lane >> 4) * 16;                                            \
  ep.load_inputs(inB, 1);                                                                                          \
  _Pragma("unroll 1") for (int q = 0; q < 4; ++q) {                                                                \
    switch (q) {                                                                                                   \
      case 0: EPIL_DUMP_ROW(acc00, acc01, 0, 0) EPIL_DUMP_ROW(acc00, acc01, 1, 16 * EPIL_PITCH) break;             \
      case 1: EPIL_DUMP_ROW(acc00, acc01, 2, 0) EPIL_DUMP_ROW(acc00, acc01, 3, 16 * EPIL_PITCH) break;             \
      case 2: EPIL_DUMP_ROW(acc10, acc11, 0, 0) EPIL_DUMP_ROW(acc10, acc11, 1, 16 * EPIL_PITCH) break;             \
      default: EPIL_DUMP_ROW(acc10, acc11, 2, 0) EPIL_DUMP_ROW(acc10, acc11, 3, 16 * EPIL_PITCH) break;            \
    }                                                                                                              \
    ep.process(inA, 2 * q, 0);                                                                                     \
    ep.load_inputs(inA, q < 3 ? 2 * q + 2 : 7);                                                                    \
    ep.process(inB, 2 * q + 1, 16 * EPIL_PITCH);                                                                   \
    ep.load_inputs(inB, q < 3 ? 2 * q + 3 : 7);                                                                    \
  }

template <bool OUT_F32, bool RES, int AUX, bool GROUPED = false>
__global__ __launch_bounds__(GEMM_THREADS, 1) void vlm_gemm_big_kernel(const gemm_params_t p_in) {
  __shared__ __attribute__((aligned(1024))) unsigned char sA0[BIG_OP_BYTES], sA1[BIG_OP_BYTES], sB0[BIG_OP_BYTES], sB1[BIG_OP_BYTES];
  __shared__ __attribute__((aligned(16))) unsigned char epl[4 * EPIL_WAVE_BYTES];
  const int tid = threadIdx.x;
  const int lane = tid & 63;
  const int wave = __builtin_amdgcn_readfirstlane(tid >> 6);
  const int wm = wave >> 1, wn = wave & 1;

  const uint32_t nblk = gridDim.x, bid = blockIdx.x;
  const uint32_t q8 = nblk >> 3, r8 = nblk & 7, xcd = bid & 7;
  const uint32_t tile = (xcd < r8 ? xcd * (q8 + 1) : r8 * (q8 + 1) + (xcd - r8) * q8) + (bid >> 3);
  uint32_t tm, tn;
  {
    const uint32_t gm = (uint32_t)p_in.group_m, gsz = gm * p_in.tiles_n, grp = tile / gsz, first = grp * gm;
    const uint32_t rows = min(gm, (uint32_t)p_in.tiles_m - first), in = tile - grp * gsz;
    tm = first + in % rows;
    tn = in / rows;
  }
  gemm_params_t p_grp;
  uint32_t m0 = tm * BIG_BM, tm_ws = tm;
  if constexpr (GROUPED) {
    p_grp = p_in;
    int g = 0;
#pragma unroll
    for (int i = 1; i < VLM_GEMM_MAX_GROUPS; ++i)
      if (i < p_in.n_groups && tm >= (uint32_t)p_in.grp[i].tile0) g = i;
    const gemm_group_t G = p_in.grp[g];
    tm_ws = tm - (uint32_t)G.tile0;
    m0 = (uint32_t)G.row0 + tm_ws * BIG_BM;
    p_grp.M = G.row_end;
    p_grp.B = G.B;
    p_grp.ldb = G.ldb;
    p_grp.epi.bias = G.bias;
    p_grp.epi.col_sum = G.col_sum;
    p_grp.epi.col_sum_ws = G.col_sum_ws;
  }
  const gemm_params_t& p = GROUPED ? p_grp : p_in;
  GEMM_STAMP(0)
  const uint32_t n0 = tn * BIG_BN;
  const __amdgpu_buffer_rsrc_t ra =
      __builtin_amdgcn_make_buffer_rsrc(const_cast<void*>(p.A), 0, (int)((uint64_t)p.M * p.lda * 2), 0x00020000);
  const __amdgpu_buffer_rsrc_t rb =
      __builtin_amdgcn_make_buffer_rsrc(const_cast<void*>(p.B), 0, (int)((uint64_t)p.N * p.ldb * 2), 0x00020000);

  uint32_t offa[4], offb[4];
  {
    const uint32_t chunk = (lane & 3) ^ big_swz(lane >> 4);
#pragma unroll
    for (int u = 0; u < 4; ++u) {
      const uint32_t row = (wave + 4 * u) * 16 + (lane >> 2);
      offa[u] = ((m0 + row) * (uint32_t)p.lda + chunk * 8) * 2;
      offb[u] = ((n0 + row) * (uint32_t)p.ldb + chunk * 8) * 2;
    }
  }
  const uint32_t rd_slot = ((uint32_t)(lane >> 4) ^ big_swz((lane & 15) >> 2)) * 16 + (lane & 15) * 64;
  const uint32_t rda = wm * 128 * 64 + rd_slot, rdb = wn * 128 * 64 + rd_slot;

  f32x4 acc00[4][4], acc01[4][4], acc10[4][4], acc11[4][4];
#pragma unroll
  for (int i = 0; i < 4; ++i)
#pragma unroll
    for (int j = 0; j < 4; ++j) {
      acc00[i][j] = (f32x4){0.f, 0.f, 0.f, 0.f};
      acc01[i][j] = (f32x4){0.f, 0.f, 0.f, 0.f};
      acc10[i][j] = (f32x4){0.f, 0.f, 0.f, 0.f};
      acc11[i][j] = (f32x4){0.f, 0.f, 0.f, 0.f};
    }

#define BIG_PIN_ACC()                                                                                   \
  _Pragma("unroll") for (int i = 0; i < 4; ++i) _Pragma("unroll") for (int j = 0; j < 4; ++j) {         \
    asm volatile("" : "+a"(acc00[i][j]), "+a"(acc01[i][j]), "+a"(acc10[i][j]), "+a"(acc11[i][j]));      \
  }
  constexpr bool DEEP = AUX == 2 && !RES;
  constexpr int AHEAD = 6;
  if constexpr (DEEP) { BIG_PIN_ACC() }

  const int nk = p.K / BIG_BK;
  const uint32_t mw0 = m0 + wm * 128, nw0 = n0 + wn * 128;
  unsigned char* const wl = epl + wave * EPIL_WAVE_BYTES;
#define EPIL_SETUP()                                       \
  big_epilogue_t<OUT_F32, RES, AUX> ep(p, wl, mw0, nw0, lane); \
  epil_in_t inA, inB;                                      \
  ep.load_inputs(inA, 0);
  bf16x8 fa0[8], fb0[8], fa1[8], fb1[8];

#define BIG_READ(FA, FB, SA, SB)                                                         \
  _Pragma("unroll") for (int i = 0; i < 8; ++i) {                                        \
    FA[i] = *reinterpret_cast<const bf16x8*>((SA) + rda + i * 1024);                     \
    FB[i] = *reinterpret_cast<const bf16x8*>((SB) + rdb + i * 1024);                     \
  }
#define BIG_MFMA_Q(ACC, FA, FB, I0, J0)                                                                                \
  _Pragma("unroll") for (int i = 0; i < 4; ++i) _Pragma("unroll") for (int j = 0; j < 4; ++j)                         \
      ACC[i][j] = __builtin_amdgcn_mfma_f32_16x16x32_bf16(FB[(J0) + j], FA[(I0) + i], ACC[i][j], 0, 0, 0);
#define BIG_MFMA(FA, FB)        \
  BIG_MFMA_Q(acc00, FA, FB, 0, 0) \
  BIG_MFMA_Q(acc01, FA, FB, 0, 4) \
  BIG_MFMA_Q(acc11, FA, FB, 4, 4) \
  BIG_MFMA_Q(acc10, FA, FB, 4, 0)
  uint32_t wr_off[4];
  {
    const uint32_t slot = (lane & 3) ^ big_swz(lane >> 4);
#pragma unroll
    for (int u = 0; u < 4; ++u) wr_off[u] = ((wave + 4 * u) * 16 + (lane >> 2)) * 64 + slot * 16;
  }
  {
    const uint32_t unswz = (((lane & 3) ^ big_swz(lane >> 4)) - (lane & 3)) * 16;
#pragma unroll
    for (int u = 0; u < 4; ++u) { offa[u] -= unswz; offb[u] -= unswz; }
  }
  u32x4 ra0[4], rb0[4], ra1[4], rb1[4];
#define BIG_GLOAD(RA_, RB_, S)                                                                        \
  _Pragma("unroll") for (int u = 0; u < 4; ++u) {                                                     \
    RA_[u] = __builtin_amdgcn_raw_buffer_load_b128(ra, offa[u], (S) * (BIG_BK * 2), 0);               \
    RB_[u] = __builtin_amdgcn_raw_buffer_load_b128(rb, offb[u], (S) * (BIG_BK * 2), 0);               \
  }
#define BIG_LWRITE(RA_, RB_, SA, SB)                                                                  \
  _Pragma("unroll") for (int u = 0; u < 4; ++u) {                                                     \
    *reinterpret_cast<u32x4*>((SA) + wr_off[u]) = RA_[u];                                             \
    *reinterpret_cast<u32x4*>((SB) + wr_off[u]) = RB_[u];                                             \
  }
#define BIG_STEP(K, GL, WR, RD, FCA, FCB, FNA, FNB, RSA, RSB, BUFA_W, BUFB_W, BUFA_R, BUFB_R)   \
  {                                                                                      \
    if (RD) {                                                                            \
      asm volatile("s_waitcnt lgkmcnt(0)" ::: "memory");                                 \
      __builtin_amdgcn_s_barrier();                                                      \
    }                                                                                    \
    __builtin_amdgcn_sched_barrier(0);                                                   \
    if (WR) { BIG_LWRITE(RSA, RSB, BUFA_W, BUFB_W) }                                     \
    if (GL) { BIG_GLOAD(RSA, RSB, (K) + 4) }                                             \
    if (RD) { BIG_READ(FNA, FNB, BUFA_R, BUFB_R) }                                       \
    BIG_MFMA(FCA, FCB)                                                                   \
    _Pragma("unroll") for (int g = 0; g < 16; ++g) {                                     \
      __builtin_amdgcn_sched_group_barrier(0x008, 2, 0);                                 \
      __builtin_amdgcn_sched_group_barrier(0x100, 1, 0);                                 \
    }                                                                                    \
    _Pragma("unroll") for (int g = 0; g < 8; ++g) {                                      \
      __builtin_amdgcn_sched_group_barrier(0x008, 2, 0);                                 \
      __builtin_amdgcn_sched_group_barrier(0x200, 1, 0);                                 \
      __builtin_amdgcn_sched_group_barrier(0x008, 2, 0);                                 \
      __builtin_amdgcn_sched_group_barrier(0x020, 1, 0);                                 \
    }                                                                                    \
    __builtin_amdgcn_sched_barrier(0);                                                   \
  }

  BIG_GLOAD(ra0, rb0, 0)
  BIG_GLOAD(ra1, rb1, 1)
  BIG_LWRITE(ra0, rb0, sA0, sB0)
  BIG_GLOAD(ra0, rb0, 2)
  BIG_LWRITE(ra1, rb1, sA1, sB1)
  BIG_GLOAD(ra1, rb1, 3)
  asm volatile("s_waitcnt lgkmcnt(0)" ::: "memory");
  __builtin_amdgcn_s_barrier();
  BIG_READ(fa0, fb0, sA0, sB0)
  GEMM_STAMP(1)

  int kt = 0;
  for (; kt < nk - 4; kt += 2) {
    BIG_STEP(kt + 0, 1, 1, 1, fa0, fb0, fa1, fb1, ra0, rb0, sA0, sB0, sA1, sB1)
    BIG_STEP(kt + 1, 1, 1, 1, fa1, fb1, fa0, fb0, ra1, rb1, sA1, sB1, sA0, sB0)
  }
#define BIG_TAIL_STEPS()                                                               \
  BIG_STEP(kt + 0, 0, 1, 1, fa0, fb0, fa1, fb1, ra0, rb0, sA0, sB0, sA1, sB1)          \
  BIG_STEP(kt + 1, 0, 1, 1, fa1, fb1, fa0, fb0, ra1, rb1, sA1, sB1, sA0, sB0)          \
  BIG_STEP(kt + 2, 0, 0, 1, fa0, fb0, fa1, fb1, ra0, rb0, sA0, sB0, sA1, sB1)          \
  BIG_STEP(kt + 3, 0, 0, 0, fa1, fb1, fa0, fb0, ra1, rb1, sA1, sB1, sA0, sB0)
  if constexpr (DEEP) {
    BIG_TAIL_STEPS()
    GEMM_STAMP(2)
    big_epilogue_t<OUT_F32, RES, AUX> ep(p, wl, mw0, nw0, lane);
    float* ws_row = (p.epi.col_sum_ws && mw0 + 128 <= (uint32_t)p.M) ? p.epi.col_sum_ws + ((size_t)(tm_ws * 2 + wm) * 2) * p.N : nullptr;
    BIG_EPILOGUE_LOOP_DEEP(AHEAD)
    ep.finish(lane, ws_row);
  } else {
    EPIL_SETUP()
    BIG_TAIL_STEPS()
    GEMM_STAMP(2)
    float* ws_row = (p.epi.col_sum_ws && mw0 + 128 <= (uint32_t)p.M) ? p.epi.col_sum_ws + ((size_t)(tm_ws * 2 + wm) * 2) * p.N : nullptr;
    BIG_EPILOGUE_LOOP()
    ep.finish(lane, ws_row);
  }
  GEMM_STAMP_END()
}

template <bool GROUPED = false>
__global__ __launch_bounds__(GEMM_THREADS, 1) void vlm_gemm_bigT_kernel(const gemm_params_t p) {
  __shared__ __attribute__((aligned(1024))) unsigned char sA0[BIG_OP_BYTES], sA1[BIG_OP_BYTES], sB0[BIG_OP_BYTES], sB1[BIG_OP_BYTES];
  __shared__ __attribute__((aligned(16))) unsigned char epl[4 * EPIL_WAVE_BYTES];
  const int tid = threadIdx.x;
  const int lane = tid & 63;
  const int wave = __builtin_amdgcn_readfirstlane(tid >> 6);
  const int wm = wave >> 1, wn = wave & 1;
  uint32_t ntile = p.tiles_m * p.tiles_n, tiles_n = (uint32_t)p.tiles_n;
  const uint32_t q8 = gridDim.x >> 3, r8 = gridDim.x & 7, xcd = blockIdx.x & 7;
  uint32_t item = (xcd < r8 ? xcd * (q8 + 1) : r8 * (q8 + 1) + (xcd - r8) * q8) + (blockIdx.x >> 3);
  uint32_t k_base = 0, k_end = (uint32_t)p.K, ws_base = 0;
  int nk = p.ksteps_per_split;
  const void *A = p.A, *B = p.B;
  uint32_t lda = (uint32_t)p.lda, ldb = (uint32_t)p.ldb;
  int M = p.M, N = p.N;
  if constexpr (GROUPED) {
    int g = 0;
#pragma unroll
    for (int i = 1; i < VLM_GEMM_MAX_GROUPS; ++i)
      if (i < p.n_groups && item >= (uint32_t)p.grpT[i].item0) g = i;
    const gemmT_group_t G = p.grpT[g];
    item -= (uint32_t)G.item0;
    k_base = (uint32_t)G.row0;
    k_end = (uint32_t)G.row_end;
    nk = G.kps;
    ws_base = G.ws_base;
    A = G.A; B = G.B;
    lda = (uint32_t)G.lda; ldb = (uint32_t)G.ldb;
    M = G.M; N = G.N;
    ntile = (uint32_t)G.ntile; tiles_n = (uint32_t)G.tiles_n;
  }
  const uint32_t split = item / ntile, tile = item - split * ntile;
  const uint32_t tm = tile / tiles_n, tn = tile - tm * tiles_n;
  const uint32_t m0 = tm * BIG_BM, n0 = tn * BIG_BN;
  const uint32_t k_first = k_base + split * (uint32_t)nk * BIG_BK;
  const __amdgpu_buffer_rsrc_t ra =
      __builtin_amdgcn_make_buffer_rsrc(const_cast<void*>(A), 0, (int)((uint64_t)k_end * lda * 2), 0x00020000);
  const __amdgpu_buffer_rsrc_t rb =
      __builtin_amdgcn_make_buffer_rsrc(const_cast<void*>(B), 0, (int)((uint64_t)k_end * ldb * 2), 0x00020000);

  uint32_t offa[4], offb[4], wr_off[4];
#pragma unroll
  for (int u = 0; u < 4; ++u) {
    const uint32_t row = 2 * (wave + 4 * u) + (lane >> 5), c16 = lane & 31;
    offa[u] = ((k_first + row) * lda + m0 + c16 * 8) * 2;
// ... 136 lines not shown
         (!e->col_scale || ((uintptr_t)e->col_scale & 15) == 0);
}

static bool epi_off32(const vlm_epilogue_t* e, int M, int lda, int ldc) {
  return (uint64_t)M * ldc * 4 < (1ull << 31) && (!e->residual || (uint64_t)M * e->ld_res * 4 < (1ull << 31)) &&
         (!e->aux || (uint64_t)M * e->ld_aux * 2 < (1ull << 31)) && (uint64_t)M * lda * 2 < (1ull << 31);
}

static int launch_gemm_bigT(gemm_params_t p, const vlm_epilogue_t* epi, hipStream_t stream) {
  if (!epi->splitk_ws || (p.N % BIG_BN) || (p.ldc % 4)) return 1;
  if ((uint64_t)p.M * p.N * 4 >= (1ull << 31)) return 1;
  p.tiles_m = (p.M + BIG_BM - 1) / BIG_BM;
  p.tiles_n = (p.N + BIG_BN - 1) / BIG_BN;
  const int ntile = p.tiles_m * p.tiles_n, nk = (p.K + BIG_BK - 1) / BIG_BK;
  int splits = plan_cus() / ntile;
  if (splits < 1) splits = 1;
  if (splits > nk / 16) splits = nk / 16;
  if (splits < 1) return 1;
  int kps = (nk + splits - 1) / splits;
  kps += kps & 1;
  if (kps < 4) kps = 4;
  splits = (nk + kps - 1) / kps;
  if ((size_t)splits * p.M * p.N * 4 > (size_t)epi->splitk_ws_bytes) return 1;
  p.ksteps_per_split = kps;
  p.splits = splits;
  float* const out = reinterpret_cast<float*>(p.C);
  const int ldc = p.ldc;
  p.C = epi->splitk_ws;
  hipLaunchKernelGGL(vlm_gemm_bigT_kernel<false>, dim3(ntile * splits), dim3(GEMM_THREADS), 0, stream, p);
  VLM_CHECK_LAUNCH();
  const size_t per = (size_t)p.M * p.N / 4;
  hipLaunchKernelGGL(splitk_reduce_kernel, dim3((unsigned)((per + 255) / 256)), dim3(256), 0, stream,
                     reinterpret_cast<const float*>(epi->splitk_ws), splits, p.M, p.N, out, ldc, epi->accumulate);
  VLM_CHECK_LAUNCH();
  return VLM_OK;
}

template <bool OUT_F32, bool RES, int AUX, bool GROUPED = false>
static int launch_gemm_big(gemm_params_t p, hipStream_t stream) {
  if (!GROUPED) p.tiles_m = (p.M + BIG_BM - 1) / BIG_BM;
  p.tiles_n = (p.N + BIG_BN - 1) / BIG_BN;
  p.group_m = p.tiles_n >= 6 ? 4 : 1;
  GEMM_STAMP_ARM(p)
  hipLaunchKernelGGL((vlm_gemm_big_kernel<OUT_F32, RES, AUX, GROUPED>), dim3(p.tiles_m * p.tiles_n), dim3(GEMM_THREADS), 0, stream, p);
  VLM_CHECK_LAUNCH();
  return VLM_OK;
}

template <bool GROUPED = false>
static int launch_gemm_big_variant(const gemm_params_t& p, bool c_is_f32, hipStream_t s) {
  const vlm_epilogue_t& e = p.epi;
  const bool res = e.residual != nullptr;
  const int aux = e.aux ? ((e.act == VLM_ACT_GELU_BWD || e.act == VLM_ACT_MUL_AUX) ? 2 : 1) : 0;
  if (e.row_scale && !res) return 1;
  {
    bool any_cs = e.col_sum != nullptr;
    if (GROUPED)
      for (int g = 0; g < p.n_groups; ++g) any_cs = any_cs || p.grp[g].col_sum != nullptr;
    if (e.alpha != 1.0f || (e.col_scale && !res) || (any_cs && aux != 2)) return 1;
  }
  if (!c_is_f32 && !res) {
    if (aux == 0) return launch_gemm_big<false, false, 0, GROUPED>(p, s);
    if (aux == 1) return launch_gemm_big<false, false, 1, GROUPED>(p, s);
    return launch_gemm_big<false, false, 2, GROUPED>(p, s);
  }
  if (c_is_f32 && aux != 2) {
    if (res && aux) return launch_gemm_big<true, true, 1, GROUPED>(p, s);
    if (res) return launch_gemm_big<true, true, 0, GROUPED>(p, s);
    if (GROUPED) return 1;
    if (aux == 0) return launch_gemm_big<true, false, 0>(p, s);
  }
  return 1;
}

static std::atomic<int> g_big_mode{1};
static int gemm_big_mode() { return g_big_mode.load(std::memory_order_relaxed); }
extern "C" int vlm_gemm_set_big_tile_mode(int mode) {
  if (mode < -1 || mode > 2) return VLM_ERR_ARG;
  g_big_mode.store(mode < 0 ? 1 : mode, std::memory_order_relaxed);
  return VLM_OK;
}


extern "C" int vlm_gemm_bf16(int ta, int tb, int M, int N, int K, const void* A, int lda, const void* B, int ldb,
                             void* C, int ldc, int c_is_f32, const vlm_epilogue_t* epi, void* stream) {
  if (M < 0 || N < 0 || K < 0 || !C) return VLM_ERR_ARG;
  if (M == 0 || N == 0) return VLM_OK;
  if (!A || !B || !epi) return VLM_ERR_ARG;
  if ((lda & 7) || (ldb & 7) || ((uintptr_t)A & 15) || ((uintptr_t)B & 15)) return VLM_ERR_ARG;
  if ((!ta || !tb) && (K % GEMM_BK)) return VLM_ERR_UNSUPPORTED;
  if (((ldc & 3) == 0) && ((uintptr_t)C & 15)) return VLM_ERR_ARG;
  if (epi->accumulate && !c_is_f32) return VLM_ERR_ARG;
  if ((epi->act == VLM_ACT_GELU_BWD || epi->act == VLM_ACT_MUL_AUX || epi->act == VLM_ACT_GELU_DERIV) && !epi->aux) return VLM_ERR_ARG;
  if (epi->act < VLM_ACT_NONE || epi->act > VLM_ACT_MUL_AUX) return VLM_ERR_ARG;
  if (epi->col_sum_ws && (!epi->col_sum || (N % GEMM_BN) != 0 || ta)) return VLM_ERR_ARG;
  const uint64_t a_bytes = (uint64_t)(ta ? K : M) * lda * 2, b_bytes = (uint64_t)(tb ? K : N) * ldb * 2;
  if (a_bytes >= (1ull << 31) || b_bytes >= (1ull << 31)) return VLM_ERR_UNSUPPORTED;
  gemm_params_t p;
  p.A = A; p.B = B; p.C = C;
  p.M = M; p.N = N; p.K = K;
  p.lda = lda; p.ldb = ldb; p.ldc = ldc;
  p.epi = *epi;
  p.epi.reserved = epi_vec8(epi, ldc, c_is_f32) ? 1 : 0;
  if (epi->col_sum_ws && !p.epi.reserved) return VLM_ERR_ARG;
  p.tiles_m = (M + GEMM_BM - 1) / GEMM_BM;
  p.tiles_n = (N + GEMM_BN - 1) / GEMM_BN;
  p.splits = 1;
  p.ksteps_per_split = 0;
  p.n_groups = 0;
  p.group_m = p.tiles_n >= 12 ? 8 : 1;
  GEMM_STAMP_ARM(p)
  hipStream_t s = (hipStream_t)stream;
  const int ntile = p.tiles_m * p.tiles_n, nk = (K + GEMM_BK - 1) / GEMM_BK;
  const bool plain_acc = epi->accumulate && c_is_f32 && !epi->bias && !epi->col_scale && !epi->row_scale &&
                         !epi->residual && !epi->aux && !epi->col_sum && epi->act == VLM_ACT_NONE;
  if (gemm_big_mode() > 0 && ta && tb && c_is_f32 && !epi->bias && !epi->col_scale && !epi->row_scale && !epi->residual &&
      !epi->aux && !epi->col_sum && epi->act == VLM_ACT_NONE && K >= 2048) {
    const int rc = launch_gemm_bigT(p, epi, s);
    if (rc <= 0) return rc;
  }
  if (tb && plain_acc && ntile < 512 && nk >= 32) {
    int splits = 2 * plan_cus() / ntile;
    if (splits < 1) splits = 1;
    if (splits > nk / 8) splits = nk / 8;
    if (splits > 1) {
      p.ksteps_per_split = (nk + splits - 1) / splits;
      p.splits = (nk + p.ksteps_per_split - 1) / p.ksteps_per_split;
      p.group_m = p.tiles_n >= 12 ? 1 : 4;
      if (ta) return launch_gemm<true, true, true, true>(p, s);
      return launch_gemm<false, true, true, true>(p, s);
    }
  }
  if (!ta && !tb && (K % (4 * BIG_BK)) == 0 && gemm_big_mode() > 0) {
    const long big_tiles = (long)((M + BIG_BM - 1) / BIG_BM) * ((N + BIG_BN - 1) / BIG_BN);
    const bool ws_ok = (N % BIG_BN) == 0 && p.epi.reserved == 1 && epi_off32(epi, M, lda, ldc) && !epi->accumulate;
    if (ws_ok && (gemm_big_mode() >= 2 || 2 * big_tiles >= plan_cus())) {
      const int rc = launch_gemm_big_variant<>(p, c_is_f32 != 0, s);
      if (rc <= 0) return rc;
    }
  }
#ifdef GEMM_ONLY_BIG
  return VLM_ERR_UNSUPPORTED;
#endif
  const int key = (ta ? 4 : 0) | (tb ? 2 : 0) | (c_is_f32 ? 1 : 0);
  switch (key) {
    case 0: return launch_gemm<false, false, false, false>(p, s);
    case 1: return launch_gemm<false, false, true, false>(p, s);
    case 2: return launch_gemm<false, true, false, false>(p, s);
    case 3: return launch_gemm<false, true, true, false>(p, s);
    case 4: return launch_gemm<true, false, false, false>(p, s);
    case 5: return launch_gemm<true, false, true, false>(p, s);
    case 6: return launch_gemm<true, true, false, false>(p, s);
    default: return launch_gemm<true, true, true, false>(p, s);
  }
}

extern "C" int vlm_gemm_bf16_grouped(int n_groups, const vlm_gemm_group_t* groups, int N, int K, const void* A, int lda, void* C,
                                     int ldc, int c_is_f32, const vlm_epilogue_t* epi, void* stream) {
  if (n_groups < 1 || n_groups > VLM_GEMM_MAX_GROUPS || !groups || N < 0 || K < 0 || !C || !epi) return VLM_ERR_ARG;
  if (epi->bias || epi->col_sum || epi->col_sum_ws || epi->splitk_ws) return VLM_ERR_ARG;
  int prev_end = 0;
  for (int g = 0; g < n_groups; ++g) {
    const vlm_gemm_group_t& G = groups[g];
    if (G.row0 < prev_end || G.rows < 0 || !G.B || (G.col_sum_ws && !G.col_sum)) return VLM_ERR_ARG;
    prev_end = G.row0 + G.rows;
  }
  const int M_total = prev_end;
  if (M_total == 0 || N == 0) return VLM_OK;
  if (!A) return VLM_ERR_ARG;
  hipStream_t s = (hipStream_t)stream;
  bool big = gemm_big_mode() > 0 && (K % (4 * BIG_BK)) == 0 && (N % BIG_BN) == 0 && !epi->accumulate && (lda & 7) == 0 &&
             ((uintptr_t)A & 15) == 0 && ((uintptr_t)C & 15) == 0 && epi_vec8(epi, ldc, c_is_f32) && epi_off32(epi, M_total, lda, ldc);
  gemm_params_t p;
  p.A = A; p.B = nullptr; p.C = C;
  p.M = M_total; p.N = N; p.K = K;
  p.lda = lda; p.ldb = 0; p.ldc = ldc;
  p.epi = *epi;
  p.epi.reserved = 1;
  p.splits = 1;
  p.ksteps_per_split = 0;
  p.n_groups = 0;
  int tiles = 0;
  for (int g = 0; g < n_groups && big; ++g) {
    const vlm_gemm_group_t& G = groups[g];
    if (G.rows == 0) continue;
    if ((G.ldb & 7) || ((uintptr_t)G.B & 15) || (uint64_t)N * G.ldb * 2 >= (1ull << 31) || (G.bias && ((uintptr_t)G.bias & 15))) big = false;
    gemm_group_t& D = p.grp[p.n_groups++];
    D.B = G.B; D.bias = G.bias; D.col_sum = G.col_sum; D.col_sum_ws = G.col_sum_ws;
    D.ldb = G.ldb; D.row0 = G.row0; D.row_end = G.row0 + G.rows; D.tile0 = tiles;
    tiles += (G.rows + BIG_BM - 1) / BIG_BM;
  }
  if (big && p.n_groups >= 1) {
    p.tiles_m = tiles;
    if (gemm_big_mode() >= 2 || 2l * tiles * (N / BIG_BN) >= plan_cus()) {
      const int rc = launch_gemm_big_variant<true>(p, c_is_f32 != 0, s);
      if (rc <= 0) return rc;
    }
  }
  for (int g = 0; g < n_groups; ++g) {
    const vlm_gemm_group_t& G = groups[g];
    if (G.rows == 0) continue;
    vlm_epilogue_t e = *epi;
    const size_t r0 = (size_t)G.row0;
    e.bias = G.bias; e.col_sum = G.col_sum; e.col_sum_ws = G.col_sum_ws;
    if (e.residual) e.residual += r0 * e.ld_res;
    if (e.aux) e.aux = reinterpret_cast<unsigned char*>(e.aux) + r0 * e.ld_aux * 2;
    if (e.row_scale) e.row_scale += r0;
    const int rc = vlm_gemm_bf16(0, 0, G.rows, N, K, reinterpret_cast<const unsigned char*>(A) + r0 * lda * 2, lda, G.B, G.ldb,
                                 reinterpret_cast<unsigned char*>(C) + r0 * ldc * (c_is_f32 ? 4 : 2), ldc, c_is_f32, &e, stream);
    if (rc) return rc;
  }
  return VLM_OK;
}

struct wgradT_problem_t {
  const void* A;
  const void* B;
  int lda, ldb, M, N, row0, row_end;
  float* C;
  int ldc, accumulate;
};
static int launch_gemm_bigT_grouped(int n, const wgradT_problem_t* pr, float* splitk_ws, uint64_t splitk_ws_bytes, hipStream_t s) {
  if (!splitk_ws || ((uintptr_t)splitk_ws & 15) || n < 1 || n > VLM_GEMM_MAX_GROUPS) return 1;
  wgrad_plan_in_t in[VLM_GEMM_MAX_GROUPS];
  for (int g = 0; g < n; ++g) {
    const wgradT_problem_t& P = pr[g];
    if (P.M < 1 || P.N < 1 || (P.N % BIG_BN) || (P.ldc % 4) || P.ldc < P.N || ((uintptr_t)P.C & 15) || ((uintptr_t)P.A & 15) ||
        ((uintptr_t)P.B & 15) || (P.lda & 7) || (P.ldb & 7) || P.lda < P.M || P.ldb < P.N || P.row0 < 0 || P.row_end <= P.row0)
      return 1;
    if ((uint64_t)P.M * P.N * 4 >= (1ull << 31) || (uint64_t)P.row_end * P.lda * 2 >= (1ull << 31) ||
        (uint64_t)P.row_end * P.ldb * 2 >= (1ull << 31))
      return 1;
    in[g] = wgrad_plan_in_t{((P.M + BIG_BM - 1) / BIG_BM) * (P.N / BIG_BN), (P.row_end - P.row0 + BIG_BK - 1) / BIG_BK,
                            (uint64_t)P.M * P.N};
  }
  wgrad_plan_t plan;
  if (wgrad_plan(n, in, plan_cus(), splitk_ws_bytes / 4, &plan)) return 1;
// ... 89 lines not shown
```

### vl-merging_amd/engine.py

```python
import itertools
import math
import os
import weakref
from typing import List, Optional

import torch

from . import _lib as L
from . import ops

BF16, F32 = torch.bfloat16, torch.float32
ALIGN = 64


def _touch_hook(p):
    p._vlm_flat.touched.add(p._vlm_name)


def touch(*params):
    for p in params:
        if p is not None:
            f = getattr(p, "_vlm_flat", None)
            if f is not None:
                f.touched.add(p._vlm_name)
# ... 135 lines not shown
        side = wgrad_stream()
        if side is None:
            ops.layerscale_finish(jobs)
        else:
            side.wait_stream(torch.cuda.current_stream())
            with torch.cuda.stream(side):
                ops.layerscale_finish(jobs)
            if not _WGRAD["pending"]:
                torch.cuda.current_stream().wait_stream(side)
        for i in layers:
            pend.discard(i)

    def zero_grad(self):
        self.flat_g.zero_()
        if getattr(self, "ls_pending", None) or getattr(self, "_ls_armed", False):
            for jobs in getattr(self, "_ls_jobs", {}).values():
                for j in jobs:
                    j["raw_w"].zero_()
                    if j["raw_b"] is not None:
                        j["raw_b"].zero_()
            self.ls_pending.clear()
            self._ls_armed = False

    def slice_of(self, names):
        lo = min(self.offsets[n][0] for n in names)
        hi = max(self.offsets[n][0] + self.extent[n] for n in names)
        return lo, hi


_WGRAD = {"stream": None, "enabled": os.environ.get("VLM_WGRAD_STREAM", "1") != "0", "pending": False}


def wgrad_stream():
    if not _WGRAD["enabled"]:
        return None
    if _WGRAD["stream"] is None:
        _WGRAD["stream"] = torch.cuda.Stream()
    return _WGRAD["stream"]


def sync_wgrad():
    if _WGRAD["stream"] is not None:
        torch.cuda.current_stream().wait_stream(_WGRAD["stream"])
    _WGRAD["pending"] = False


def _arm_wgrad_join():
    if not _WGRAD["pending"]:
        _WGRAD["pending"] = True
        torch.autograd.Variable._execution_engine.queue_callback(sync_wgrad)


class _Side:

    def __init__(self, *tensors):
        self.s = wgrad_stream()
        self.tensors = tensors
        self.ctx = None

    def __enter__(self):
        if self.s is None:
            return self
        self.s.wait_stream(torch.cuda.current_stream())
        for t in self.tensors:
            t.record_stream(self.s)
        _arm_wgrad_join()
        self.ctx = torch.cuda.stream(self.s)
        self.ctx.__enter__()
        return self

    def __exit__(self, *a):
        if self.ctx is not None:
            self.ctx.__exit__(*a)
        return False


def wT16(p):
    s = getattr(p, "_vlm_bf16_t", None)
    if s is None:
        raise L.VlmError("weight has no transposed bf16 shadow: call model.setup_engine() on a CUDA model first")
    return s


def _gemm_rows(a, groups, out, *, act=L.ACT_NONE, aux=None, col_scale=None, row_scale=None, residual=None, col_sum_fold=None):
    if len(groups) > 1:
        return ops.gemm_grouped(a, groups, out, act=act, aux=aux, col_scale=col_scale, row_scale=row_scale,
                                residual=residual, col_sum_fold=col_sum_fold)
    (r0, r1, w, bias, col_sum), = groups

    def rows(t):
        return t[r0:r1] if t is not None else None

    return ops.gemm(a[r0:r1], w, out[r0:r1], bias=bias, act=act, aux=rows(aux), col_scale=col_scale,
                    row_scale=rows(row_scale), residual=rows(residual), col_sum=col_sum, col_sum_fold=col_sum_fold)


def _wgrad_rows(dy, x, groups):
    if len(groups) > 1:
        return ops.gemm_wgrad_grouped(dy, x, groups)
    (r0, r1, dw), = groups
    return ops.gemm(dy[r0:r1], x[r0:r1], dw, ta=True, tb=True, accumulate=True)


def w16(p):
    s = getattr(p, "_vlm_bf16", None)
    if s is None:
        raise L.VlmError("parameter has no bf16 shadow: call model.setup_engine() on a CUDA model first")
    return s


class RelPos:

    def __init__(self, bias_t, index16, index16_t, holder, cache_tag=None, cache=None):
        self.bias_t = bias_t
        self.index = index16
        self.index_t = index16_t
        self.holder = holder
        self._dense = {}
        self.cache_tag = cache_tag
        self.cache = cache

    def dense_for(self, seq, mode):
        key = (seq.n0, seq.n1, seq.pos1, mode)
        d = self._dense.get(key)
        if d is None:
            ck = self.cache_tag + key if self.cache_tag is not None and self.cache is not None else None
            cache = self.cache
            d = cache.get(ck) if ck is not None else None
            if d is None:
                with torch.no_grad():
                    d = ops.bias_dense(self.bias_t.detach(), self.index, seq, mode)
                _DENSE_STATS["built"] += 1
                if ck is not None:
                    for k in [k for k in cache if k[:2] != ck[:2]]:
                        del cache[k]
                    while len(cache) >= 8:
                        del cache[next(iter(cache))]
                    cache[ck] = d
            else:
                _DENSE_STATS["hits"] += 1
            self._dense[key] = d
        return d

    @property
    def dbias_t(self):
        return self.holder["dbias_t"]


_CONSTS = {}
CONST_MAX = 64


def const(key, build):
    t = _CONSTS.get(key)
    if t is None:
        if len(_CONSTS) >= CONST_MAX:
            del _CONSTS[next(iter(_CONSTS))]
        t = _CONSTS[key] = build()
    return t


_ZERO = {}


def _zero_scalar(dev):
    z = _ZERO.get(str(dev))
    if z is None:
        z = _ZERO[str(dev)] = torch.zeros((), device=dev, dtype=F32)
    return z


class _TableT(torch.autograd.Function):

    @staticmethod
    def forward(ctx, table, holder):
        ctx.holder, ctx.table = holder, table
        flat = getattr(table, "_vlm_flat", None)
# ... 148 lines not shown
            continue
        lo, hi = base, base + seq.B * n
        owner = [e for r0, r1, e in ranges if r0 <= lo and hi <= r1]
        if len(owner) != 1:
            return None, None, False
        if owner[0].qb is not None:
            qb[sgm], vb[sgm] = owner[0].qb.grad, owner[0].vb.grad
    return qb, vb, True


class BlockPlan:

    def __init__(self, ranges, mode, gamma1, gamma2, layer, drop_prob, eps):
        self.ranges = ranges
        self.mode = mode
        self.gamma1, self.gamma2 = gamma1, gamma2
        self.layer = layer
        self.drop_prob = drop_prob
        self.eps = eps


def _qkv_bias(e):
    if e.qb is None:
        return None
    view = getattr(e.qb, "_vlm_qkv_bias", None)
    if view is not None:
        return view
    return torch.cat((e.qb.detach(), torch.zeros_like(e.vb), e.vb.detach()))


_FOLD_LS = os.environ.get("VLM_FOLD_LAYERSCALE", "1") != "0"


def _folded(ranges):
    return _FOLD_LS and all(getattr(e.projw, "_vlm_raw", None) is not None and getattr(e.fc2w, "_vlm_raw", None) is not None
                            for _, _, e in ranges)


def _fb(b):
    return b._vlm_folded if b is not None else None


def _rb(b):
    return b._vlm_raw if b is not None else None


def _arm_layerscale_finish(flat):
    if getattr(flat, "_ls_armed", False):
        return
    flat._ls_armed = True

    def done():
        flat._ls_armed = False
        flat.finish_layerscale()
        sync_wgrad()

    torch.autograd.Variable._execution_engine.queue_callback(done)


def _ln2_bwd_scale1(dln, x1, st2, e, dx1, dx2, y1, g1, rs1, dy1, fold):
    sgamma, dsgamma, dsbias = (None, None, _rb(e.projb)) if y1 is None else (g1, g1.grad, e.projb.grad)
    if x1.shape[1] <= 768:
        ops.layernorm_bwd_scale(dln, x1, st2, e.n2w, dx1, dx2, e.n2w.grad, e.n2b.grad, y=y1, sgamma=sgamma, row_scale=rs1,
                                sdy=dy1, dsgamma=dsgamma, dsbias=dsbias, fold=fold)
    else:
        ops.layernorm_bwd(dln, x1, st2, e.n2w, dx1, dres=dx2, dgamma=e.n2w.grad, dbeta=e.n2b.grad, fold=fold)
        ops.layerscale_bwd(dx1, y1, sgamma, rs1, dy1, dsgamma, dsbias, fold=fold)


class _BlockFn(torch.autograd.Function):

    @staticmethod
    def forward(ctx, x, bias_t, plan: BlockPlan, pc: PassCtx, training: bool, hook):
        M, D = x.shape
        dev = x.device
        H = pc.H
        Fdim = plan.ranges[0][2].fc1w.shape[0]
        x = x.contiguous()
        ln1 = torch.empty(M, D, device=dev, dtype=BF16)
        st1 = torch.empty(M, 2, device=dev, dtype=F32)
        qkv = torch.empty(M, 3 * D, device=dev, dtype=BF16)
        rs1 = pc.drop_path_rows(plan.drop_prob, training, dev)
        rs2 = pc.drop_path_rows(plan.drop_prob, training, dev)
        rg = plan.ranges
        for r0, r1, e in rg:
            ops.layernorm_fwd(x[r0:r1], e.n1w, e.n1b, plan.eps, ln1[r0:r1], st1[r0:r1])
        _gemm_rows(ln1, [(r0, r1, w16(e.qkvw), _qkv_bias(e), None) for r0, r1, e in rg], qkv)
        o = torch.empty(M, D, device=dev, dtype=BF16)
        lse = torch.empty(H, M, device=dev, dtype=F32)
        rp = pc.relpos
        ops.attention_fwd(qkv, o, lse, pc.seq, H, bias_t=bias_t, head_row0=plan.layer * H,
                          rel_index=rp.index if rp is not None else None,
                          rel_index_t=rp.index_t if rp is not None else None, keep0=pc.keep0, keep1=pc.keep1,
                          mode=plan.mode, bias_dense=rp.dense_for(pc.seq, plan.mode) if rp is not None else None)
        x1 = torch.empty(M, D, device=dev, dtype=F32)
        folded = _folded(plan.ranges)
        y1 = torch.empty(M, D, device=dev, dtype=BF16) if not folded else None
        ln2 = torch.empty(M, D, device=dev, dtype=BF16)
        st2 = torch.empty(M, 2, device=dev, dtype=F32)
        h = torch.empty(M, Fdim, device=dev, dtype=BF16)
        a = torch.empty(M, Fdim, device=dev, dtype=BF16)
        x2 = torch.empty(M, D, device=dev, dtype=F32)
        y2 = torch.empty(M, D, device=dev, dtype=BF16) if not folded else None
        cs1, cs2 = (None, None) if folded else (plan.gamma1, plan.gamma2)
        pb = (lambda e: _fb(e.projb)) if folded else (lambda e: e.projb)
        fb2 = (lambda e: _fb(e.fc2b)) if folded else (lambda e: e.fc2b)
        _gemm_rows(o, [(r0, r1, w16(e.projw), pb(e), None) for r0, r1, e in rg], x1, col_scale=cs1, row_scale=rs1,
                   residual=x, aux=y1)
        for r0, r1, e in rg:
            ops.layernorm_fwd(x1[r0:r1], e.n2w, e.n2b, plan.eps, ln2[r0:r1], st2[r0:r1])
        _gemm_rows(ln2, [(r0, r1, w16(e.fc1w), e.fc1b, None) for r0, r1, e in rg], a, act=L.ACT_GELU_DERIV, aux=h)
        _gemm_rows(a, [(r0, r1, w16(e.fc2w), fb2(e), None) for r0, r1, e in rg], x2, col_scale=cs2, row_scale=rs2,
                   residual=x1, aux=y2)
        if pc.gram is not None:
            for r0, r1, e in plan.ranges:
                gn = e.gram_names
                if gn.get("qkv") or gn.get("fc1"):
                    t32 = torch.empty(r1 - r0, D, device=dev, dtype=F32)
                    st = torch.empty(r1 - r0, 2, device=dev, dtype=F32)
                    if gn.get("qkv"):
                        ops.layernorm_fwd(x[r0:r1], e.n1w, e.n1b, plan.eps, t32, st)
                        pc.gram.add(gn.get("qkv"), t32)
                    if gn.get("fc1"):
                        ops.layernorm_fwd(x1[r0:r1], e.n2w, e.n2b, plan.eps, t32, st)
                        pc.gram.add(gn.get("fc1"), t32)
                pc.gram.add(gn.get("proj"), o[r0:r1])
                pc.gram.add(gn.get("fc2"), a[r0:r1])
        ctx.plan, ctx.pc, ctx.hook = plan, pc, hook
        ctx.has_bias = bias_t is not None
        ctx.folded = folded
        ctx.save_for_backward(x, st1, ln1, qkv, o, lse, y1 if y1 is not None else x.new_empty(0), x1, st2, ln2, h, a,
                              y2 if y2 is not None else x.new_empty(0),
                              rs1 if rs1 is not None else x.new_empty(0), rs2 if rs2 is not None else x.new_empty(0),
                              bias_t if bias_t is not None else x.new_empty(0))
        return x2

    @staticmethod
    def backward(ctx, dx2):
        plan, pc = ctx.plan, ctx.pc
        x, st1, ln1, qkv, o, lse, y1, x1, st2, ln2, h, a, y2, rs1, rs2, bias_t = ctx.saved_tensors
        rs1 = rs1 if rs1.numel() else None
        rs2 = rs2 if rs2.numel() else None
        bias_t = bias_t if ctx.has_bias else None
        M, D = x.shape
        dev = x.device
        H = pc.H
        Fdim = h.shape[1]
        dx2 = dx2.contiguous()
        g1, g2 = plan.gamma1, plan.gamma2
        folded = ctx.folded
        if folded:
            y1 = y2 = None
            flat = plan.ranges[0][2].projw._vlm_flat
            _arm_layerscale_finish(flat)
        wg = (lambda w: w._vlm_raw) if folded else (lambda w: w.grad)
        touch(g1, g2)
        for _, _, e in plan.ranges:
            _touch_expert(e)
        dy2 = torch.empty(M, D, device=dev, dtype=BF16)
        dy1 = torch.empty(M, D, device=dev, dtype=BF16)
        dh = torch.empty(M, Fdim, device=dev, dtype=BF16)
        dln = torch.empty(M, D, device=dev, dtype=BF16)
        dx1 = torch.empty(M, D, device=dev, dtype=F32)
        fold = ops.FoldBatch(dev, D)
        rg = plan.ranges
        do = torch.empty(M, D, device=dev, dtype=BF16)
        for r0, r1, e in rg:
            rr = slice(r0, r1)
            if folded:
                ops.layerscale_bwd(dx2[rr], None, None, rs2[rr] if rs2 is not None else None, dy2[rr], None, _rb(e.fc2b), fold=fold)
            else:
                ops.layerscale_bwd(dx2[rr], y2[rr], g2, rs2[rr] if rs2 is not None else None, dy2[rr], g2.grad, e.fc2b.grad,
                                   fold=fold)
        _gemm_rows(dy2, [(r0, r1, wT16(e.fc2w), None, e.fc1b.grad) for r0, r1, e in rg], dh, act=L.ACT_MUL_AUX, aux=h,
                   col_sum_fold=fold)
        batch = wgrad_stream() is not None and len(rg) == 1 and ops.wgrad_batch_serves(
            rg[0][1] - rg[0][0], [(D, Fdim), (Fdim, D), (D, D), (3 * D, D)])
        if not batch:
            with _Side(dy2, a, dh, ln2):
                _wgrad_rows(dy2, a, [(r0, r1, wg(e.fc2w)) for r0, r1, e in rg])
                _wgrad_rows(dh, ln2, [(r0, r1, e.fc1w.grad) for r0, r1, e in rg])
        _gemm_rows(dh, [(r0, r1, wT16(e.fc1w), None, None) for r0, r1, e in rg], dln)
        for r0, r1, e in rg:
            rr = slice(r0, r1)
            _ln2_bwd_scale1(dln[rr], x1[rr], st2[rr], e, dx1[rr], dx2[rr], y1[rr] if y1 is not None else None, g1,
                            rs1[rr] if rs1 is not None else None, dy1[rr], fold)
        _gemm_rows(dy1, [(r0, r1, wT16(e.projw), None, None) for r0, r1, e in rg], do)
        if not batch:
            with _Side(dy1, o):
                _wgrad_rows(dy1, o, [(r0, r1, wg(e.projw)) for r0, r1, e in rg])
        dqkv = torch.empty(M, 3 * D, device=dev, dtype=BF16)
        dln1 = torch.empty(M, D, device=dev, dtype=BF16)
        rp = pc.relpos
        qb_grads, vb_grads, fused_qv = _segment_bias_grads(rg, pc.seq)
        ops.attention_bwd(qkv, o, do, lse, dqkv, pc.seq, H, bias_t=bias_t, head_row0=plan.layer * H,
                          rel_index=rp.index if rp is not None else None,
                          rel_index_t=rp.index_t if rp is not None else None, keep0=pc.keep0, keep1=pc.keep1,
                          mode=plan.mode, dbias_t=rp.holder.get("dbias_t") if rp is not None else None,
                          dq_colsum=qb_grads, dv_colsum=vb_grads,
                          bias_dense=rp.dense_for(pc.seq, plan.mode) if rp is not None else None)
        dx = torch.empty(M, D, device=dev, dtype=F32)
        for r0, r1, e in rg:
            if e.qb is not None and not fused_qv:
                ops.colsum(dqkv[r0:r1, :D], e.qb.grad)
                ops.colsum(dqkv[r0:r1, 2 * D:], e.vb.grad)
        if batch:
            (r0, r1, e), = rg
            rr = slice(r0, r1)
            with _Side(dy2, a, dh, ln2, dy1, o, dqkv, ln1):
                ops.gemm_wgrad_batch([(dy2[rr], a[rr], wg(e.fc2w)), (dh[rr], ln2[rr], e.fc1w.grad),
                                      (dy1[rr], o[rr], wg(e.projw)), (dqkv[rr], ln1[rr], e.qkvw.grad)])
        else:
            with _Side(dqkv, ln1):
                _wgrad_rows(dqkv, ln1, [(r0, r1, e.qkvw.grad) for r0, r1, e in rg])
        _gemm_rows(dqkv, [(r0, r1, wT16(e.qkvw), None, None) for r0, r1, e in rg], dln1)
        for r0, r1, e in rg:
            rr = slice(r0, r1)
            ops.layernorm_bwd(dln1[rr], x[rr], st1[rr], e.n1w, dx[rr], dres=dx1[rr], dgamma=e.n1w.grad, dbeta=e.n1b.grad,
                              fold=fold)
        fold.flush()
        if folded:
            flat.ls_pending.add(plan.layer)
        if ctx.hook is not None:
            ctx.hook(plan.layer)
        dbias = None
        if bias_t is not None and ctx.needs_input_grad[1] and rp is not None and not rp.holder.get("routed"):
            rp.holder["routed"] = True
            dbias = _zero_scalar(dev).expand_as(bias_t)
        return dx, dbias, None, None, None, None


def run_block(x, plan: BlockPlan, pc: PassCtx, training: bool, hook=None):
    bias_t = pc.relpos.bias_t if pc.relpos is not None else None
    return _BlockFn.apply(x, bias_t, plan, pc, training, hook)


def _kernel_rows(t, dtypes=(BF16, F32), row_align=1, ptr_align=1, layout=True):
    if not (torch.is_tensor(t) and t.is_cuda and t.dtype in dtypes):
        return False
    return not layout or (t.dim() == 2 and t.stride(1) == 1 and t.stride(0) % row_align == 0 and t.data_ptr() % ptr_align == 0)


def _rows2d(g, D, dtypes=(BF16, F32), contiguous=False):
    g2 = g.reshape(-1, D)
    if g2.dtype not in dtypes:
        g2 = g2.float()
    return g2.contiguous() if contiguous or g2.stride(1) != 1 else g2


class _LinearFn(torch.autograd.Function):

    @staticmethod
    def forward(ctx, x, weight, bias, act):
        x2 = x.reshape(-1, x.shape[-1])
        if x2.dtype != BF16:
            x2 = x2.to(BF16)
        if x2.stride(1) != 1 or (x2.shape[0] > 1 and x2.stride(0) < x2.shape[1]):
            x2 = x2.contiguous()
        M, K = x2.shape
        N = weight.shape[0]
        Np = (N + 63) // 64 * 64
        gelu = act == "gelu"
        buf = torch.empty(M, Np, device=x.device, dtype=BF16)
        pre = torch.empty(M, Np, device=x.device, dtype=BF16) if gelu else None
        ops.gemm(x2, w16(weight), buf[:, :N], bias=bias, act=L.ACT_GELU if gelu else L.ACT_NONE,
                 aux=pre[:, :N] if gelu else None)
        y = ops.tanh_fwd(buf[:, :N]) if act == "tanh" else None
        ctx.save_for_backward(x2, pre if gelu else (y if y is not None else x2.new_empty(0)))
        ctx.weight, ctx.bias, ctx.act, ctx.shape, ctx.N, ctx.Np = weight, bias, act, x.shape, N, Np
        return (y if y is not None else buf[:, :N]).view(*x.shape[:-1], N)

    @staticmethod
    def backward(ctx, gy):
        x2, saved = ctx.saved_tensors
        weight, bias, N, Np, act = ctx.weight, ctx.bias, ctx.N, ctx.Np, ctx.act
        M, K = x2.shape
        gy2 = _rows2d(gy, N)
        if (act is None and gy2.dtype == BF16 and gy2.stride() == (Np, 1) and gy2.storage_offset() == 0
                and _is_padded_grad(gy2, M, Np)):
            dy = torch.as_strided(gy2, (M, Np), (Np, 1))
        elif act is None and Np == N and gy2.dtype == BF16:
            dy = gy2
        else:
            mode = {"gelu": ops.ACT_BWD_GELU, "tanh": ops.ACT_BWD_TANH, None: ops.ACT_BWD_NONE}[act]
            dy = ops.act_bwd(gy2, saved[:, :N] if act is not None else None, mode, Np)
        touch(weight if weight.requires_grad else None, bias if bias is not None and bias.requires_grad else None)
        if bias is not None and bias.requires_grad:
            if N % 8 == 0:
                ops.colsum(dy[:, :N], bias.grad)
            elif N <= 64:
                ops.colsum_small(dy[:, :N], bias.grad)
            elif bias.grad.is_contiguous():
                N8 = N // 8 * 8
                ops.colsum(dy[:, :N8], bias.grad[:N8])
                ops.colsum_small(dy[:, N8:N], bias.grad[N8:])
            else:
                bias.grad.add_(dy[:, :N].float().sum(0))
        if weight.requires_grad:
# ... 397 lines not shown
```

### vl-merging_amd/ops.py

```python
import ctypes

import torch

from . import _lib as L

BF16 = torch.bfloat16
F32 = torch.float32


def _ld(t):
    if t.dim() != 2 or t.stride(1) != 1:
        raise L.VlmError("expected a 2-D tensor with unit inner stride, got shape %s strides %s"
                         % (tuple(t.shape), t.stride()))
    return t.stride(0) if t.shape[0] > 1 else max(t.stride(0), t.shape[1])


_SCRATCH = {}


def _scratch(kind, floats, device):
    key = (kind, device.index, torch.cuda.current_stream().cuda_stream)
    ws = _SCRATCH.get(key)
    if ws is None or ws.numel() < floats:
        ws = _SCRATCH[key] = torch.empty(floats, device=device, dtype=F32)
    return ws


SPLITK_WS_BYTES = 96 << 20


def _epilogue(N, *, bias=None, col_scale=None, row_scale=None, residual=None, aux=None, act=L.ACT_NONE, alpha=1.0, accumulate=False,
              col_sum=None):
    e = L.Epilogue()
    e.bias = bias.data_ptr() if bias is not None else 0
    e.col_scale = col_scale.data_ptr() if col_scale is not None else 0
    e.row_scale = row_scale.data_ptr() if row_scale is not None else 0
    e.residual = residual.data_ptr() if residual is not None else 0
    e.ld_res = _ld(residual) if residual is not None else 0
    e.aux = aux.data_ptr() if aux is not None else 0
    e.ld_aux = _ld(aux) if aux is not None else 0
    e.act = act
    e.alpha = alpha
    e.accumulate = 1 if accumulate else 0
    e.col_sum = col_sum.data_ptr() if col_sum is not None else 0
    if col_sum is not None and (col_sum.numel() < N or not col_sum.is_contiguous()):
        raise L.VlmError("gemm: col_sum must be a contiguous f32 vector of at least N elements")
    for t, dt in ((bias, F32), (col_scale, F32), (row_scale, F32), (residual, F32), (aux, BF16), (col_sum, F32)):
        if t is not None and t.dtype != dt:
            raise L.VlmError("gemm epilogue tensor has dtype %s, expected %s" % (t.dtype, dt))
    return e


def gemm(a, b, out, ta=False, tb=False, *, bias=None, act=L.ACT_NONE, aux=None, col_scale=None, row_scale=None,
         residual=None, alpha=1.0, accumulate=False, col_sum=None, col_sum_fold=None):
    L.require_cuda(a, b, out, bias, aux, col_scale, row_scale, residual, col_sum)
    if a.dtype != BF16 or b.dtype != BF16:
        raise L.VlmError("gemm operands must be bfloat16")
    M, N = out.shape
    K = a.shape[0] if ta else a.shape[1]
    if (a.shape[1] if ta else a.shape[0]) != M:
        raise L.VlmError("gemm: A rows %s do not match M=%d" % (tuple(a.shape), M))
    kb, nb = (b.shape[0], b.shape[1]) if tb else (b.shape[1], b.shape[0])
    if nb != N or kb != K:
        raise L.VlmError("gemm: B shape %s incompatible with N=%d K=%d" % (tuple(b.shape), N, K))
    e = _epilogue(N, bias=bias, col_scale=col_scale, row_scale=row_scale, residual=residual, aux=aux, act=act, alpha=alpha,
                  accumulate=accumulate, col_sum=col_sum)
    region = None
    if col_sum is not None and col_sum_fold is not None and not ta and N % 128 == 0 and M >= 128:
        region = col_sum_fold.next_region()
        if region.numel() >= (M // 128) * 2 * N:
            e.col_sum_ws = region.data_ptr()
        else:
            region = None
    if ta and tb and out.dtype == F32 and K >= 2048 and bias is None and col_sum is None:
        ws = _scratch("splitk", SPLITK_WS_BYTES // 4, out.device)
        e.splitk_ws = ws.data_ptr()
        e.splitk_ws_bytes = ws.numel() * 4
    if out.dtype not in (BF16, F32):
        raise L.VlmError("gemm output must be bf16 or f32")
    rc = L.get_lib().vlm_gemm_bf16(int(ta), int(tb), M, N, K, L.ptr(a), _ld(a), L.ptr(b), _ld(b), L.ptr(out), _ld(out),
                                   int(out.dtype == F32), ctypes.byref(e), L.stream_ptr())
    L.check(rc, "vlm_gemm_bf16")
    if region is not None:
        col_sum_fold.add(region, M // 128, N, col_sum, None)
    return out


def gemm_grouped(a, groups, out, *, act=L.ACT_NONE, aux=None, col_scale=None, row_scale=None, residual=None, alpha=1.0,
                 col_sum_fold=None):
    L.require_cuda(a, out, aux, col_scale, row_scale, residual)
    if a.dtype != BF16:
        raise L.VlmError("gemm operands must be bfloat16")
    if len(groups) < 1 or len(groups) > L.GEMM_MAX_GROUPS:
        raise L.VlmError("gemm_grouped: 1..%d groups" % L.GEMM_MAX_GROUPS)
    M, N = out.shape
    K = a.shape[1]
    if a.shape[0] != M:
        raise L.VlmError("gemm_grouped: A rows %s do not match M=%d" % (tuple(a.shape), M))
    e = _epilogue(N, col_scale=col_scale, row_scale=row_scale, residual=residual, aux=aux, act=act, alpha=alpha)
    if out.dtype not in (BF16, F32):
        raise L.VlmError("gemm output must be bf16 or f32")
    arr = (L.GemmGroup * len(groups))()
    folds = []
    prev = 0
    if col_sum_fold is not None and len(col_sum_fold.jobs) + len(groups) > col_sum_fold.MAX:
        col_sum_fold.flush()
    for g, (r0, r1, w, bias, col_sum) in zip(arr, groups):
        L.require_cuda(w, bias, col_sum)
        if w.dtype != BF16 or tuple(w.shape) != (N, K) or r0 < prev or r1 < r0 or r1 > M:
            raise L.VlmError("gemm_grouped: group (%d, %d) weight %s for N=%d K=%d M=%d" % (r0, r1, tuple(w.shape), N, K, M))
        prev = r1
        for t in (bias, col_sum):
            if t is not None and (t.dtype != F32 or t.numel() < N or not t.is_contiguous()):
                raise L.VlmError("gemm_grouped: bias / col_sum must be contiguous f32 vectors of at least N elements")
        g.row0, g.rows, g.B, g.ldb = r0, r1 - r0, w.data_ptr(), _ld(w)
        g.bias = bias.data_ptr() if bias is not None else None
        g.col_sum = col_sum.data_ptr() if col_sum is not None else None
        rows = r1 - r0
        if col_sum is not None and col_sum_fold is not None and N % 128 == 0 and rows >= 128:
            region = col_sum_fold.next_region()
            if region.numel() >= (rows // 128) * 2 * N:
                g.col_sum_ws = region.data_ptr()
                col_sum_fold.add(region, rows // 128, N, col_sum, None)
                folds.append(region)
    rc = L.get_lib().vlm_gemm_bf16_grouped(len(groups), arr, N, K, L.ptr(a), _ld(a), L.ptr(out), _ld(out),
                                           int(out.dtype == F32), ctypes.byref(e), L.stream_ptr())
    L.check(rc, "vlm_gemm_bf16_grouped")
    return out


def gemm_wgrad_grouped(dy, x, groups, accumulate=True):
    L.require_cuda(dy, x)
    if dy.dtype != BF16 or x.dtype != BF16 or dy.shape[0] != x.shape[0]:
        raise L.VlmError("gemm_wgrad_grouped: bf16 dy [tokens, M] and x [tokens, N]")
    M, N = dy.shape[1], x.shape[1]
    arr = (L.WgradGroup * len(groups))()
    prev, ldc = 0, None
    for g, (r0, r1, dW) in zip(arr, groups):
        L.require_cuda(dW)
        if dW.dtype != F32 or tuple(dW.shape) != (M, N) or r0 < prev or r1 < r0 or r1 > dy.shape[0]:
            raise L.VlmError("gemm_wgrad_grouped: group (%d, %d) gradient %s for M=%d N=%d" % (r0, r1, tuple(dW.shape), M, N))
        if ldc is not None and _ld(dW) != ldc:
            raise L.VlmError("gemm_wgrad_grouped: the groups' gradients must share one leading dimension")
        ldc = _ld(dW)
        prev = r1
        g.row0, g.rows, g.C, g.accumulate = r0, r1 - r0, dW.data_ptr(), int(bool(accumulate))
    ws = _scratch("splitk", SPLITK_WS_BYTES // 4, dy.device)
    rc = L.get_lib().vlm_gemm_wgrad_grouped(len(groups), arr, M, N, L.ptr(dy), _ld(dy), L.ptr(x), _ld(x), ldc, L.ptr(ws),
                                            ws.numel() * 4, L.stream_ptr())
    L.check(rc, "vlm_gemm_wgrad_grouped")


def wgrad_batch_serves(T, shapes):
    cus = L.get_lib().vlm_device_cus()
    return (T >= 2048 and 1 <= len(shapes) <= L.GEMM_MAX_GROUPS and all(N % 256 == 0 for _, N in shapes)
            and sum(-(-M // 256) * (N // 256) for M, N in shapes) <= (cus if cus > 0 else 256))


def gemm_wgrad_batch(problems, accumulate=True):
    n = len(problems)
    if n < 1 or n > L.GEMM_MAX_GROUPS:
        raise L.VlmError("gemm_wgrad_batch: 1..%d problems" % L.GEMM_MAX_GROUPS)
    acc = [bool(accumulate)] * n if isinstance(accumulate, (bool, int)) else [bool(f) for f in accumulate]
    if len(acc) != n:
# ... 607 lines not shown
    d.ld_qkv = _ld(qkv)
    d.H = H
    d.total_rows = qkv.shape[0]
    if bias_t is not None:
        if bias_t.dtype != F32 or not bias_t.is_contiguous():
            raise L.VlmError("attention bias_t must be contiguous f32")
        if rel_index_t is None or rel_index_t.dtype != torch.int16:
            raise L.VlmError("attention needs the transposed int16 relative index (rel_index_t)")
        d.R = bias_t.shape[1]
        d.bias_t = bias_t.data_ptr()
        d.rel_index_t = rel_index_t.data_ptr()
        d.ld_index_t = _ld(rel_index_t)
        d.index_t_rows = rel_index_t.shape[0]
        if rel_index is not None:
            if rel_index.dtype != torch.int16:
                raise L.VlmError("rel_index must be int16")
            d.rel_index = rel_index.data_ptr()
            d.ld_index = _ld(rel_index)
            d.index_rows = rel_index.shape[0]
    d.head_row0 = head_row0
    d.mode = mode
    for k in (keep0, keep1):
        if k is not None and (k.dtype != torch.uint8 or not k.is_contiguous()):
            raise L.VlmError("attention keep masks must be contiguous uint8")
    d.keep0 = keep0.data_ptr() if keep0 is not None else 0
    d.keep1 = keep1.data_ptr() if keep1 is not None else 0
    d.B, d.n0, d.n1, d.base0, d.base1, d.pos1 = seq.B, seq.n0, seq.n1, seq.base0, seq.base1, seq.pos1
    d.scale = scale
    if bias_t is not None:
        if bias_dense is None:
            if rel_index is None:
                raise L.VlmError("attention with a bias needs bias_dense (ops.bias_dense) or the int16 index")
            bias_dense = globals()["bias_dense"](bias_t, rel_index, seq, mode)
        if not isinstance(bias_dense, DenseBias) or bias_dense.key != (seq.n0, seq.n1, seq.pos1, mode):
            raise L.VlmError("bias_dense must come from ops.bias_dense() for the same geometry and mode")
        d.bias_dense, d.bias_dense_t = bias_dense.q_major.data_ptr(), bias_dense.k_major.data_ptr()
        d.dense_tiles = bias_dense.tiles
        d._keep = bias_dense
    return d


class DenseBias:

    __slots__ = ("q_major", "k_major", "tiles", "key")

    def __init__(self, q_major, k_major, tiles, key):
        self.q_major, self.k_major, self.tiles, self.key = q_major, k_major, tiles, key


def bias_dense(bias_t, index16, seq, mode):
    L.require_cuda(bias_t, index16)
    if index16.dtype != torch.int16 or not index16.is_contiguous() or index16.shape[0] < seq.pos1 + seq.n1:
        raise L.VlmError("bias_dense: contiguous int16 index with pos1 + n1 rows")
    if bias_t.dtype != F32 or not bias_t.is_contiguous():
        raise L.VlmError("bias_dense: contiguous f32 bias_t [n_cols, R]")
    n_cols, R = bias_t.shape
    nbytes = L.get_lib().vlm_bias_dense_bytes(seq.n0, seq.n1, seq.pos1, mode)
    if nbytes == 0:
        raise L.VlmError("bias_dense: bad geometry (pos1 %% 8 == 0, pos1 >= n0)")
    outs = []
    for k_major in (0, 1):
        flat = torch.empty(n_cols * (nbytes // 2) + 8192, device=bias_t.device, dtype=torch.float16)
        out = flat[: n_cols * (nbytes // 2)].view(n_cols, nbytes // 2)
        L.check(L.get_lib().vlm_bias_dense(L.ptr(bias_t), n_cols, R, L.ptr(index16), _ld(index16), seq.n0, seq.n1, seq.pos1,
                                           mode, k_major, L.ptr(out), L.stream_ptr()), "vlm_bias_dense")
        outs.append(out)
    return DenseBias(outs[0], outs[1], nbytes // 4096, (seq.n0, seq.n1, seq.pos1, mode))


def attention_fwd(qkv, out, lse, seq, H, *, bias_t=None, head_row0=0, rel_index=None, rel_index_t=None, keep0=None,
                  keep1=None, mode=L.ATTN_JOINT, scale=0.125, bias_dense=None):
    d = _attn_desc(qkv, seq, H, bias_t, head_row0, rel_index, rel_index_t, keep0, keep1, mode, scale, bias_dense)
    L.require_cuda(out, lse)
    rc = L.get_lib().vlm_attention_fwd(ctypes.byref(d), L.ptr(out), _ld(out), L.ptr(lse), L.stream_ptr())
    L.check(rc, "vlm_attention_fwd")
    return out


_ATTN_WS = {}


def attention_bwd(qkv, out, dout, lse, dqkv, seq, H, *, bias_t=None, head_row0=0, rel_index=None, rel_index_t=None,
                  keep0=None, keep1=None, mode=L.ATTN_JOINT, scale=0.125, dbias_t=None, delta_ws=None,
                  dq_colsum=None, dv_colsum=None, bias_dense=None):
    d = _attn_desc(qkv, seq, H, bias_t, head_row0, rel_index, rel_index_t, keep0, keep1, mode, scale, bias_dense)
    L.require_cuda(out, dout, lse, dqkv, dbias_t, delta_ws)
    cs = None
    if dq_colsum is not None or dv_colsum is not None:
        cs = L.AttnColsum()
        for name, pair in (("dq", dq_colsum), ("dv", dv_colsum)):
            for sgm, t in enumerate(pair or (None, None)):
                if t is not None:
                    L.require_cuda(t)
                    if t.dtype != F32 or t.numel() < H * 64 or not t.is_contiguous():
                        raise L.VlmError("attention_bwd: column-sum outputs must be contiguous f32 [H*64]")
                    getattr(cs, name)[sgm] = t.data_ptr()
    need = L.get_lib().vlm_attention_bwd_ws_floats(ctypes.byref(d), 0)
    if delta_ws is None or delta_ws.numel() < need:
        key = (qkv.device.index, torch.cuda.current_stream().cuda_stream)
        delta_ws = _ATTN_WS.get(key)
        if delta_ws is None or delta_ws.numel() < need:
            delta_ws = _ATTN_WS[key] = torch.empty(need, device=qkv.device, dtype=F32)
    if bias_t is not None and rel_index is None:
        raise L.VlmError("attention_bwd needs both orientations of the int16 relative index")
    rc = L.get_lib().vlm_attention_bwd(ctypes.byref(d), L.ptr(out), _ld(out), L.ptr(dout), _ld(dout), L.ptr(lse),
                                       L.ptr(delta_ws), delta_ws.numel(), L.ptr(dqkv), _ld(dqkv), L.ptr(dbias_t),
                                       ctypes.byref(cs) if cs is not None else None, L.stream_ptr())
    L.check(rc, "vlm_attention_bwd")
    return dqkv


def debug_occupy(workgroups, threads, lds_bytes, microseconds):
    L.check(L.get_lib().vlm_debug_occupy(int(workgroups), int(threads), int(lds_bytes), int(microseconds), L.stream_ptr()),
            "vlm_debug_occupy")


def _layerscale_jobs(jobs):
    for i in range(0, len(jobs), L.MAX_LAYERSCALE_JOBS):
        chunk = jobs[i:i + L.MAX_LAYERSCALE_JOBS]
        arr = (L.LayerScaleJob * len(chunk))()
        for a, j in zip(arr, chunk):
            w = j["weight"]
            L.require_cuda(w, *[v for v in j.values() if torch.is_tensor(v)])
            for f in ("weight", "gamma", "bias", "shadow", "bias_out", "raw_w", "raw_b", "dweight", "dbias", "dgamma"):
                t = j.get(f)
                setattr(a, f, t.data_ptr() if t is not None else None)
            a.N, a.K = w.shape[0], w.shape[1]
        yield arr, len(chunk)


def layerscale_fold(jobs):
    for arr, n in _layerscale_jobs(jobs):
        L.check(L.get_lib().vlm_layerscale_fold(arr, n, L.stream_ptr()), "vlm_layerscale_fold")


def layerscale_finish(jobs):
    for arr, n in _layerscale_jobs(jobs):
        L.check(L.get_lib().vlm_layerscale_finish(arr, n, L.stream_ptr()), "vlm_layerscale_finish")
```

Baseline: 351.0.

## Skip GEMM tiles and attention-backward work for drop-path-dropped rows

Passes the per-row drop-path scale vector as a liveness mask into the big-tile GEMM and the attention backward kernels. GEMM tiles whose rows all have zero scale skip the K loop and only run the epilogue on zero accumulators. Attention dQ and dK/dV work items for dead samples write zeros and the required statistics, then exit early. This targets the compute spent on samples that stochastic depth drops during training. In exchange it adds extra interfaces and branches, and it relies on dead rows contributing exactly zero downstream.

```diff
diff --git a/include/vlm_hip.h b/include/vlm_hip.h
--- a/include/vlm_hip.h
+++ b/include/vlm_hip.h
@@ -303,6 +303,8 @@
 
 int vlm_gemm_bf16(int ta, int tb, int M, int N, int K, const void* A, int lda, const void* B, int ldb, void* C,
                   int ldc, int c_is_f32, const vlm_epilogue_t* epi, void* stream);
+int vlm_gemm_bf16_live(int ta, int tb, int M, int N, int K, const void* A, int lda, const void* B, int ldb, void* C,
+                       int ldc, int c_is_f32, const vlm_epilogue_t* epi, const float* row_live, void* stream);
 #define VLM_GEMM_MAX_GROUPS 4
 typedef struct {
   int32_t row0, rows;
@@ -504,6 +506,9 @@
 int vlm_attention_bwd(const vlm_attn_desc_t* d, const void* out_bf16, int ld_out, const void* dout_bf16, int ld_dout,
                       const float* lse, float* delta_ws, size_t ws_floats, void* dqkv_bf16, int ld_dqkv, float* dbias_t,
                       const vlm_attn_colsum_t* colsum, void* stream);
+int vlm_attention_bwd_live(const vlm_attn_desc_t* d, const void* out_bf16, int ld_out, const void* dout_bf16, int ld_dout,
+                           const float* lse, float* delta_ws, size_t ws_floats, void* dqkv_bf16, int ld_dqkv, float* dbias_t,
+                           const vlm_attn_colsum_t* colsum, const float* row_live, void* stream);
 
 #ifdef __cplusplus
 }
diff --git a/vl-merging_amd/_lib.py b/vl-merging_amd/_lib.py
--- a/vl-merging_amd/_lib.py
+++ b/vl-merging_amd/_lib.py
@@ -321,6 +321,8 @@
     "vlm_sce_run": (c_int, [c_void_p, c_void_p]),
     "vlm_gemm_bf16": (c_int, [c_int, c_int, c_int, c_int, c_int, c_void_p, c_int, c_void_p, c_int, c_void_p, c_int,
                               c_int, ctypes.POINTER(Epilogue), c_void_p]),
+    "vlm_gemm_bf16_live": (c_int, [c_int, c_int, c_int, c_int, c_int, c_void_p, c_int, c_void_p, c_int, c_void_p, c_int,
+                                   c_int, ctypes.POINTER(Epilogue), c_void_p, c_void_p]),
     "vlm_gemm_bf16_grouped": (c_int, [c_int, ctypes.POINTER(GemmGroup), c_int, c_int, c_void_p, c_int, c_void_p, c_int, c_int,
                                       ctypes.POINTER(Epilogue), c_void_p]),
     "vlm_gemm_wgrad_grouped": (c_int, [c_int, ctypes.POINTER(WgradGroup), c_int, c_int, c_void_p, c_int, c_void_p, c_int, c_int,
@@ -330,6 +332,8 @@
     "vlm_attention_bwd_ws_floats": (c_size_t, [ctypes.POINTER(AttnDesc), c_int]),
     "vlm_attention_bwd": (c_int, [ctypes.POINTER(AttnDesc), c_void_p, c_int, c_void_p, c_int, c_void_p, c_void_p, c_size_t,
                                   c_void_p, c_int, c_void_p, c_void_p, c_void_p]),
+    "vlm_attention_bwd_live": (c_int, [ctypes.POINTER(AttnDesc), c_void_p, c_int, c_void_p, c_int, c_void_p, c_void_p, c_size_t,
+                                       c_void_p, c_int, c_void_p, c_void_p, c_void_p, c_void_p]),
     "vlm_layernorm_fwd": (c_int, [c_void_p, c_int, c_int, c_int, c_void_p, c_void_p, c_float, c_void_p, c_int, c_int,
                                   c_void_p, c_void_p]),
     "vlm_layernorm_bwd": (c_int, [c_void_p, c_int, c_int, c_void_p, c_int, c_void_p, c_void_p, c_int, c_int, c_void_p,
diff --git a/vl-merging_amd/csrc/attention_bwd.hip b/vl-merging_amd/csrc/attention_bwd.hip
--- a/vl-merging_amd/csrc/attention_bwd.hip
+++ b/vl-merging_amd/csrc/attention_bwd.hip
@@ -17,7 +17,15 @@
   float* nstat;
   float* dq_colsum[2];
   float* dv_colsum[2];
+  const float* row_live;
 };
+
+__device__ __forceinline__ bool att_bwd_dead(const attn_bwd_params_t& bp, const att_pos_t& ps, int part, int b) {
+  if (!bp.row_live) return false;
+  const bool d0 = ps.n0 == 0 || bp.row_live[ps.base0 + b * ps.n0] == 0.0f;
+  const bool d1 = ps.n1 == 0 || bp.row_live[ps.base1 + b * ps.n1] == 0.0f;
+  return bp.f.mode == VLM_ATTN_SEPARATE ? (part ? d1 : d0) : (d0 && d1);
+}
 
 #include "attention_bwd_dkvb.h"
 #include "attention_bwd_dq2.h"
@@ -743,10 +751,11 @@
   hipLaunchKernelGGL((attn_bwd_dkvb_kernel<W>), dim3((unsigned)((pl.items + 7) / 8 * 8)), dim3(W * 64), pl.lds, s, bp, pl.groups, pl.panel_blocks);
 }
 
-extern "C" int vlm_attention_bwd(const vlm_attn_desc_t* d, const void* out, int ld_out, const void* d_out,
-                                 int ld_dout, const float* lse, float* delta_ws, size_t ws_floats, void* dqkv, int ld_dqkv,
-                                 float* dbias_t, const vlm_attn_colsum_t* colsum, void* stream) {
+static int attention_bwd(const vlm_attn_desc_t* d, const void* out, int ld_out, const void* d_out, int ld_dout, const float* lse,
+                         float* delta_ws, size_t ws_floats, void* dqkv, int ld_dqkv, float* dbias_t, const vlm_attn_colsum_t* colsum,
+                         const float* row_live, void* stream) {
   attn_bwd_params_t bp;
+  bp.row_live = row_live;
   int rc = att_fill_params(d, bp.f);
   if (rc != VLM_OK) return rc;
   if (!out || !d_out || !lse || !delta_ws || !dqkv) return VLM_ERR_ARG;
@@ -801,3 +810,16 @@
   VLM_CHECK_LAUNCH();
   return VLM_OK;
 }
+
+extern "C" int vlm_attention_bwd(const vlm_attn_desc_t* d, const void* out, int ld_out, const void* d_out,
+                                 int ld_dout, const float* lse, float* delta_ws, size_t ws_floats, void* dqkv, int ld_dqkv,
+                                 float* dbias_t, const vlm_attn_colsum_t* colsum, void* stream) {
+  return attention_bwd(d, out, ld_out, d_out, ld_dout, lse, delta_ws, ws_floats, dqkv, ld_dqkv, dbias_t, colsum, nullptr, stream);
+}
+
+extern "C" int vlm_attention_bwd_live(const vlm_attn_desc_t* d, const void* out, int ld_out, const void* d_out,
+                                      int ld_dout, const float* lse, float* delta_ws, size_t ws_floats, void* dqkv, int ld_dqkv,
+                                      float* dbias_t, const vlm_attn_colsum_t* colsum, const float* row_live, void* stream) {
+  if (row_live && ((uintptr_t)row_live & 3)) return VLM_ERR_ARG;
+  return attention_bwd(d, out, ld_out, d_out, ld_dout, lse, delta_ws, ws_floats, dqkv, ld_dqkv, dbias_t, colsum, row_live, stream);
+}
diff --git a/vl-merging_amd/csrc/attention_bwd_dkvb.h b/vl-merging_amd/csrc/attention_bwd_dkvb.h
--- a/vl-merging_amd/csrc/attention_bwd_dkvb.h
+++ b/vl-merging_amd/csrc/attention_bwd_dkvb.h
@@ -107,7 +107,19 @@
   const int rounds = (b_hi - b_lo + wact - 1) / wact;
   for (int rd = 0; rd < rounds; ++rd) {
     const int b = b_lo + rd * wact + wave;
-    const bool active = wave < wact && b < b_hi;
+    bool active = wave < wact && b < b_hi;
+    if (active && __builtin_amdgcn_readfirstlane((int)att_bwd_dead(bp, ps, part, b)) != 0) {
+#pragma unroll
+      for (int i = 0; i < 16; ++i) {
+        const int kpi = kp0 + (i & 3) + 8 * (i >> 2) + 4 * hh;
+        const int row = kpi < s_hi ? att_row_of(ps, b, kpi) : -1;
+        if (row >= 0) {
+          bf16_t* dst = bp.dqkv + (size_t)row * bp.ld_dqkv + D + h * 64 + r;
+          dst[0] = dst[32] = dst[D] = dst[D + 32] = (bf16_t)0.f;
+        }
+      }
+      active = false;
+    }
 
     bf16x8 kf[4], vf[4], bstat;
     f32x16 dk[2], dv[2];
diff --git a/vl-merging_amd/csrc/attention_bwd_dq2.h b/vl-merging_amd/csrc/attention_bwd_dq2.h
--- a/vl-merging_amd/csrc/attention_bwd_dq2.h
+++ b/vl-merging_amd/csrc/attention_bwd_dq2.h
@@ -37,6 +37,27 @@
   if (!att_work_item(att_num_tiles(ps.n0, ps.n1, ps.pos1, p.mode), ps.B, p.H, wtile, b, h)) return;
   const att_span_t sp = att_span(ps, p.mode, wtile);
   ATT_STAMP(0);
+  if (att_bwd_dead(bp, ps, sp.part, b)) {
+    const int qpd = sp.p0 + wave * 32 + r;
+    const int rowd = qpd < sp.s_hi ? att_row_of(ps, b, qpd) : -1;
+    if (rowd >= 0) {
+      bf16_t* op = bp.dqkv + (size_t)rowd * bp.ld_dqkv + h * 64 + 4 * hh;
+      const bf16x4 z = {(bf16_t)0.f, (bf16_t)0.f, (bf16_t)0.f, (bf16_t)0.f};
+#pragma unroll
+      for (int db = 0; db < 2; ++db)
+#pragma unroll
+        for (int g4 = 0; g4 < 4; ++g4) *reinterpret_cast<bf16x4*>(op + db * 32 + 8 * g4) = z;
+      if (hh == 0) {
+        const size_t at = (size_t)h * p.total_rows + (size_t)rowd;
+        bp.delta[at] = 0.f;
+        if (bp.nstat) {
+          bp.nstat[at] = -bp.lse[at] * bp.inv_c1;
+          bp.nstat[(size_t)p.H * p.total_rows + at] = 0.f;
+        }
+      }
+    }
+    return;
+  }
   const int D = p.H * 64;
   const int ntiles = (sp.s_hi - sp.s_lo + ATT_BK - 1) / ATT_BK;
   const uint32_t lds0 = (uint32_t)(uintptr_t)(att_lds_void*)lds;
diff --git a/vl-merging_amd/csrc/gemm.hip b/vl-merging_amd/csrc/gemm.hip
--- a/vl-merging_amd/csrc/gemm.hip
+++ b/vl-merging_amd/csrc/gemm.hip
@@ -137,6 +137,7 @@
   int n_groups;
   gemm_group_t grp[VLM_GEMM_MAX_GROUPS];
   gemmT_group_t grpT[VLM_GEMM_MAX_GROUPS];
+  const float* row_live = nullptr;
   VLM_DIAG_GEMM_FIELD
 };
 
@@ -792,6 +793,17 @@
   }
   const gemm_params_t& p = GROUPED ? p_grp : p_in;
   GEMM_STAMP(0)
+  constexpr bool SKIPS = !(RES && AUX == 1);
+  f32x4 lv = {1.f, 1.f, 1.f, 1.f};
+  if (SKIPS && p.row_live) {
+    const uint32_t m = m0 + 4 * (uint32_t)lane;
+    if (m0 + BIG_BM <= (uint32_t)p.M && ((uintptr_t)p.row_live & 15) == 0) {
+      lv = *reinterpret_cast<const f32x4*>(p.row_live + m);
+    } else {
+#pragma unroll
+      for (int e = 0; e < 4; ++e) lv[e] = p.row_live[min(m + e, (uint32_t)p.M - 1)];
+    }
+  }
   const uint32_t n0 = tn * BIG_BN;
   const __amdgpu_buffer_rsrc_t ra =
       __builtin_amdgcn_make_buffer_rsrc(const_cast<void*>(p.A), 0, (int)((uint64_t)p.M * p.lda * 2), 0x00020000);
@@ -900,6 +912,23 @@
 
   BIG_GLOAD(ra0, rb0, 0)
   BIG_GLOAD(ra1, rb1, 1)
+  if (SKIPS && p.row_live && __builtin_amdgcn_ballot_w64(lv[0] != 0.0f || lv[1] != 0.0f || lv[2] != 0.0f || lv[3] != 0.0f) == 0) {
+    int lane_d = lane;
+    asm volatile("" : "+v"(lane_d));
+    big_epilogue_t<OUT_F32, RES, AUX> ep(p, wl, mw0, nw0, lane_d);
+    unsigned char* const wz = wl + (lane_d & 15) * EPIL_PITCH + (lane_d >> 4) * 16;
+#pragma unroll
+    for (int j = 0; j < 8; ++j) *reinterpret_cast<f32x4*>(wz + 64 * j) = (f32x4){0.f, 0.f, 0.f, 0.f};
+#pragma unroll 1
+    for (int i = 0; i < 8; ++i) {
+      epil_in_t in;
+      ep.load_inputs(in, i);
+      ep.process(in, i, 0);
+    }
+    ep.finish(lane_d, (p.epi.col_sum_ws && mw0 + 128 <= (uint32_t)p.M) ? p.epi.col_sum_ws + ((size_t)(tm_ws * 2 + wm) * 2) * p.N : nullptr);
+    GEMM_STAMP_END()
+    return;
+  }
   BIG_LWRITE(ra0, rb0, sA0, sB0)
   BIG_GLOAD(ra0, rb0, 2)
   BIG_LWRITE(ra1, rb1, sA1, sB1)
@@ -1202,8 +1231,8 @@
 }
 
 
-extern "C" int vlm_gemm_bf16(int ta, int tb, int M, int N, int K, const void* A, int lda, const void* B, int ldb,
-                             void* C, int ldc, int c_is_f32, const vlm_epilogue_t* epi, void* stream) {
+static int gemm_bf16(int ta, int tb, int M, int N, int K, const void* A, int lda, const void* B, int ldb, void* C, int ldc,
+                     int c_is_f32, const vlm_epilogue_t* epi, const float* row_live, void* stream) {
   if (M < 0 || N < 0 || K < 0 || !C) return VLM_ERR_ARG;
   if (M == 0 || N == 0) return VLM_OK;
   if (!A || !B || !epi) return VLM_ERR_ARG;
@@ -1255,8 +1284,10 @@
     const long big_tiles = (long)((M + BIG_BM - 1) / BIG_BM) * ((N + BIG_BN - 1) / BIG_BN);
     const bool ws_ok = (N % BIG_BN) == 0 && p.epi.reserved == 1 && epi_off32(epi, M, lda, ldc) && !epi->accumulate;
     if (ws_ok && (gemm_big_mode() >= 2 || 2 * big_tiles >= plan_cus())) {
+      p.row_live = row_live;
       const int rc = launch_gemm_big_variant<>(p, c_is_f32 != 0, s);
       if (rc <= 0) return rc;
+      p.row_live = nullptr;
     }
   }
 #ifdef GEMM_ONLY_BIG
@@ -1273,6 +1304,17 @@
     case 6: return launch_gemm<true, true, false, false>(p, s);
     default: return launch_gemm<true, true, true, false>(p, s);
   }
+}
+
+extern "C" int vlm_gemm_bf16(int ta, int tb, int M, int N, int K, const void* A, int lda, const void* B, int ldb,
+                             void* C, int ldc, int c_is_f32, const vlm_epilogue_t* epi, void* stream) {
+  return gemm_bf16(ta, tb, M, N, K, A, lda, B, ldb, C, ldc, c_is_f32, epi, nullptr, stream);
+}
+
+extern "C" int vlm_gemm_bf16_live(int ta, int tb, int M, int N, int K, const void* A, int lda, const void* B, int ldb,
+                                  void* C, int ldc, int c_is_f32, const vlm_epilogue_t* epi, const float* row_live, void* stream) {
+  if (row_live && ((uintptr_t)row_live & 3)) return VLM_ERR_ARG;
+  return gemm_bf16(ta, tb, M, N, K, A, lda, B, ldb, C, ldc, c_is_f32, epi, row_live, stream);
 }
 
 extern "C" int vlm_gemm_bf16_grouped(int n_groups, const vlm_gemm_group_t* groups, int N, int K, const void* A, int lda, void* C,
diff --git a/vl-merging_amd/engine.py b/vl-merging_amd/engine.py
--- a/vl-merging_amd/engine.py
+++ b/vl-merging_amd/engine.py
@@ -241,7 +241,17 @@
     return s
 
 
-def _gemm_rows(a, groups, out, *, act=L.ACT_NONE, aux=None, col_scale=None, row_scale=None, residual=None, col_sum_fold=None):
+_ROWSKIP = {"enabled": True}
+
+
+def _live(rs, plan, pc):
+    if not _ROWSKIP["enabled"] or pc.gram is not None or (pc.independent_segments and plan.mode == L.ATTN_JOINT):
+        return None
+    return rs
+
+
+def _gemm_rows(a, groups, out, *, act=L.ACT_NONE, aux=None, col_scale=None, row_scale=None, residual=None, col_sum_fold=None,
+               row_live=None):
     if len(groups) > 1:
         return ops.gemm_grouped(a, groups, out, act=act, aux=aux, col_scale=col_scale, row_scale=row_scale,
                                 residual=residual, col_sum_fold=col_sum_fold)
@@ -251,7 +261,8 @@
         return t[r0:r1] if t is not None else None
 
     return ops.gemm(a[r0:r1], w, out[r0:r1], bias=bias, act=act, aux=rows(aux), col_scale=col_scale,
-                    row_scale=rows(row_scale), residual=rows(residual), col_sum=col_sum, col_sum_fold=col_sum_fold)
+                    row_scale=rows(row_scale), residual=rows(residual), col_sum=col_sum, col_sum_fold=col_sum_fold,
+                    row_live=rows(row_live))
 
 
 def _wgrad_rows(dy, x, groups):
@@ -566,10 +577,11 @@
         qkv = torch.empty(M, 3 * D, device=dev, dtype=BF16)
         rs1 = pc.drop_path_rows(plan.drop_prob, training, dev)
         rs2 = pc.drop_path_rows(plan.drop_prob, training, dev)
+        live1, live2 = _live(rs1, plan, pc), _live(rs2, plan, pc)
         rg = plan.ranges
         for r0, r1, e in rg:
             ops.layernorm_fwd(x[r0:r1], e.n1w, e.n1b, plan.eps, ln1[r0:r1], st1[r0:r1])
-        _gemm_rows(ln1, [(r0, r1, w16(e.qkvw), _qkv_bias(e), None) for r0, r1, e in rg], qkv)
+        _gemm_rows(ln1, [(r0, r1, w16(e.qkvw), _qkv_bias(e), None) for r0, r1, e in rg], qkv, row_live=live1)
         o = torch.empty(M, D, device=dev, dtype=BF16)
         lse = torch.empty(H, M, device=dev, dtype=F32)
         rp = pc.relpos
@@ -590,12 +602,13 @@
         pb = (lambda e: _fb(e.projb)) if folded else (lambda e: e.projb)
         fb2 = (lambda e: _fb(e.fc2b)) if folded else (lambda e: e.fc2b)
         _gemm_rows(o, [(r0, r1, w16(e.projw), pb(e), None) for r0, r1, e in rg], x1, col_scale=cs1, row_scale=rs1,
-                   residual=x, aux=y1)
+                   residual=x, aux=y1, row_live=live1)
         for r0, r1, e in rg:
             ops.layernorm_fwd(x1[r0:r1], e.n2w, e.n2b, plan.eps, ln2[r0:r1], st2[r0:r1])
-        _gemm_rows(ln2, [(r0, r1, w16(e.fc1w), e.fc1b, None) for r0, r1, e in rg], a, act=L.ACT_GELU_DERIV, aux=h)
+        _gemm_rows(ln2, [(r0, r1, w16(e.fc1w), e.fc1b, None) for r0, r1, e in rg], a, act=L.ACT_GELU_DERIV, aux=h,
+                   row_live=live2)
         _gemm_rows(a, [(r0, r1, w16(e.fc2w), fb2(e), None) for r0, r1, e in rg], x2, col_scale=cs2, row_scale=rs2,
-                   residual=x1, aux=y2)
+                   residual=x1, aux=y2, row_live=live2)
         if pc.gram is not None:
             for r0, r1, e in plan.ranges:
                 gn = e.gram_names
@@ -625,6 +638,7 @@
         x, st1, ln1, qkv, o, lse, y1, x1, st2, ln2, h, a, y2, rs1, rs2, bias_t = ctx.saved_tensors
         rs1 = rs1 if rs1.numel() else None
         rs2 = rs2 if rs2.numel() else None
+        live1, live2 = _live(rs1, plan, pc), _live(rs2, plan, pc)
         bias_t = bias_t if ctx.has_bias else None
         M, D = x.shape
         dev = x.device
@@ -657,19 +671,19 @@
                 ops.layerscale_bwd(dx2[rr], y2[rr], g2, rs2[rr] if rs2 is not None else None, dy2[rr], g2.grad, e.fc2b.grad,
                                    fold=fold)
         _gemm_rows(dy2, [(r0, r1, wT16(e.fc2w), None, e.fc1b.grad) for r0, r1, e in rg], dh, act=L.ACT_MUL_AUX, aux=h,
-                   col_sum_fold=fold)
+                   col_sum_fold=fold, row_live=live2)
         batch = wgrad_stream() is not None and len(rg) == 1 and ops.wgrad_batch_serves(
             rg[0][1] - rg[0][0], [(D, Fdim), (Fdim, D), (D, D), (3 * D, D)])
         if not batch:
             with _Side(dy2, a, dh, ln2):
                 _wgrad_rows(dy2, a, [(r0, r1, wg(e.fc2w)) for r0, r1, e in rg])
                 _wgrad_rows(dh, ln2, [(r0, r1, e.fc1w.grad) for r0, r1, e in rg])
-        _gemm_rows(dh, [(r0, r1, wT16(e.fc1w), None, None) for r0, r1, e in rg], dln)
+        _gemm_rows(dh, [(r0, r1, wT16(e.fc1w), None, None) for r0, r1, e in rg], dln, row_live=live2)
         for r0, r1, e in rg:
             rr = slice(r0, r1)
             _ln2_bwd_scale1(dln[rr], x1[rr], st2[rr], e, dx1[rr], dx2[rr], y1[rr] if y1 is not None else None, g1,
                             rs1[rr] if rs1 is not None else None, dy1[rr], fold)
-        _gemm_rows(dy1, [(r0, r1, wT16(e.projw), None, None) for r0, r1, e in rg], do)
+        _gemm_rows(dy1, [(r0, r1, wT16(e.projw), None, None) for r0, r1, e in rg], do, row_live=live1)
         if not batch:
             with _Side(dy1, o):
                 _wgrad_rows(dy1, o, [(r0, r1, wg(e.projw)) for r0, r1, e in rg])
@@ -682,7 +696,7 @@
                           rel_index_t=rp.index_t if rp is not None else None, keep0=pc.keep0, keep1=pc.keep1,
                           mode=plan.mode, dbias_t=rp.holder.get("dbias_t") if rp is not None else None,
                           dq_colsum=qb_grads, dv_colsum=vb_grads,
-                          bias_dense=rp.dense_for(pc.seq, plan.mode) if rp is not None else None)
+                          bias_dense=rp.dense_for(pc.seq, plan.mode) if rp is not None else None, row_live=live1)
         dx = torch.empty(M, D, device=dev, dtype=F32)
         for r0, r1, e in rg:
             if e.qb is not None and not fused_qv:
@@ -697,7 +711,7 @@
         else:
             with _Side(dqkv, ln1):
                 _wgrad_rows(dqkv, ln1, [(r0, r1, e.qkvw.grad) for r0, r1, e in rg])
-        _gemm_rows(dqkv, [(r0, r1, wT16(e.qkvw), None, None) for r0, r1, e in rg], dln1)
+        _gemm_rows(dqkv, [(r0, r1, wT16(e.qkvw), None, None) for r0, r1, e in rg], dln1, row_live=live1)
         for r0, r1, e in rg:
             rr = slice(r0, r1)
             ops.layernorm_bwd(dln1[rr], x[rr], st1[rr], e.n1w, dx[rr], dres=dx1[rr], dgamma=e.n1w.grad, dbeta=e.n1b.grad,
diff --git a/vl-merging_amd/ops.py b/vl-merging_amd/ops.py
--- a/vl-merging_amd/ops.py
+++ b/vl-merging_amd/ops.py
@@ -52,8 +52,8 @@
 
 
 def gemm(a, b, out, ta=False, tb=False, *, bias=None, act=L.ACT_NONE, aux=None, col_scale=None, row_scale=None,
-         residual=None, alpha=1.0, accumulate=False, col_sum=None, col_sum_fold=None):
-    L.require_cuda(a, b, out, bias, aux, col_scale, row_scale, residual, col_sum)
+         residual=None, alpha=1.0, accumulate=False, col_sum=None, col_sum_fold=None, row_live=None):
+    L.require_cuda(a, b, out, bias, aux, col_scale, row_scale, residual, col_sum, row_live)
     if a.dtype != BF16 or b.dtype != BF16:
         raise L.VlmError("gemm operands must be bfloat16")
     M, N = out.shape
@@ -78,8 +78,14 @@
         e.splitk_ws_bytes = ws.numel() * 4
     if out.dtype not in (BF16, F32):
         raise L.VlmError("gemm output must be bf16 or f32")
-    rc = L.get_lib().vlm_gemm_bf16(int(ta), int(tb), M, N, K, L.ptr(a), _ld(a), L.ptr(b), _ld(b), L.ptr(out), _ld(out),
-                                   int(out.dtype == F32), ctypes.byref(e), L.stream_ptr())
+    if row_live is not None:
+        if row_live.dtype != F32 or row_live.dim() != 1 or row_live.shape[0] != M or row_live.stride(0) != 1:
+            raise L.VlmError("gemm: row_live must be a dense f32 vector of M=%d elements" % M)
+        rc = L.get_lib().vlm_gemm_bf16_live(int(ta), int(tb), M, N, K, L.ptr(a), _ld(a), L.ptr(b), _ld(b), L.ptr(out), _ld(out),
+                                            int(out.dtype == F32), ctypes.byref(e), L.ptr(row_live), L.stream_ptr())
+    else:
+        rc = L.get_lib().vlm_gemm_bf16(int(ta), int(tb), M, N, K, L.ptr(a), _ld(a), L.ptr(b), _ld(b), L.ptr(out), _ld(out),
+                                       int(out.dtype == F32), ctypes.byref(e), L.stream_ptr())
     L.check(rc, "vlm_gemm_bf16")
     if region is not None:
         col_sum_fold.add(region, M // 128, N, col_sum, None)
@@ -853,7 +859,7 @@
 
 def attention_bwd(qkv, out, dout, lse, dqkv, seq, H, *, bias_t=None, head_row0=0, rel_index=None, rel_index_t=None,
                   keep0=None, keep1=None, mode=L.ATTN_JOINT, scale=0.125, dbias_t=None, delta_ws=None,
-                  dq_colsum=None, dv_colsum=None, bias_dense=None):
+                  dq_colsum=None, dv_colsum=None, bias_dense=None, row_live=None):
     d = _attn_desc(qkv, seq, H, bias_t, head_row0, rel_index, rel_index_t, keep0, keep1, mode, scale, bias_dense)
     L.require_cuda(out, dout, lse, dqkv, dbias_t, delta_ws)
     cs = None
@@ -874,9 +880,15 @@
             delta_ws = _ATTN_WS[key] = torch.empty(need, device=qkv.device, dtype=F32)
     if bias_t is not None and rel_index is None:
         raise L.VlmError("attention_bwd needs both orientations of the int16 relative index")
-    rc = L.get_lib().vlm_attention_bwd(ctypes.byref(d), L.ptr(out), _ld(out), L.ptr(dout), _ld(dout), L.ptr(lse),
-                                       L.ptr(delta_ws), delta_ws.numel(), L.ptr(dqkv), _ld(dqkv), L.ptr(dbias_t),
-                                       ctypes.byref(cs) if cs is not None else None, L.stream_ptr())
+    args = (ctypes.byref(d), L.ptr(out), _ld(out), L.ptr(dout), _ld(dout), L.ptr(lse), L.ptr(delta_ws), delta_ws.numel(),
+            L.ptr(dqkv), _ld(dqkv), L.ptr(dbias_t), ctypes.byref(cs) if cs is not None else None)
+    if row_live is not None:
+        L.require_cuda(row_live)
+        if row_live.dtype != F32 or row_live.dim() != 1 or row_live.shape[0] < qkv.shape[0] or row_live.stride(0) != 1:
+            raise L.VlmError("attention_bwd: row_live must be a dense f32 vector over the rows of qkv")
+        rc = L.get_lib().vlm_attention_bwd_live(*args, L.ptr(row_live), L.stream_ptr())
+    else:
+        rc = L.get_lib().vlm_attention_bwd(*args, L.stream_ptr())
     L.check(rc, "vlm_attention_bwd")
     return dqkv
 
```

New measurement: 354.5, median of 6. 1.01x the previous value.
